# SinOncology/BreakID

Hardware: AMD Instinct MI355X
Metric: M reads/s clustered+split-scanned (higher is better)
Workload: dtype int32/u8 (+f64 sd replay)

## Files before the change

### breakid_amd/capi.py

```python
from __future__ import annotations

import ctypes as C
import math
import os
import subprocess

import numpy as np

from . import abi

_HERE = os.path.dirname(os.path.abspath(__file__))
LIB_PATH = os.path.join(_HERE, "libbreakid_hip.so")
_LIB = None


class BreakIDError(RuntimeError):
    def __init__(self, code, msg):
        super().__init__("libbreakid_hip error %d: %s" % (code, msg))
        self.code = code


def build(verbose=False):
    cmd = ["make", "-C", os.path.join(_HERE, "csrc"), "-j8"]
    r = subprocess.run(cmd, capture_output=not verbose, text=True)
    if r.returncode != 0:
        raise RuntimeError("building libbreakid_hip.so failed:\n" + (r.stdout or "")[-4000:] + (r.stderr or "")[-4000:])


EXPORTS = ["bk_init", "bk_prepare_process", "bk_free", "bk_last_error", "bk_set_stream", "bk_sync", "bk_get_stream", "bk_upload_records", "bk_records", "bk_exclude_regions", "bk_isize_stats",
           "bk_discordant_pairs", "bk_mask_and_cluster", "bk_split_evidence", "bk_cluster_summary",
           "bk_split_breakpoints", "bk_normal_support", "bk_ref_support", "bk_genotype_call", "bk_clip_support", "bk_clip_reads", "bk_base_depth", "bk_clip_rescue", "bk_junctions", "bk_junction_sides", "bk_vcf_breakend_alt", "bk_evidence", "bk_unique_support", "bk_clip_consensus", "bk_junction_fit", "bk_locus_similarity", "bk_site_complexity", "bk_window_coverage", "bk_window_context", "bk_call_windows", "bk_fusion_frame", "bk_link_calls", "bk_locus_partners", "bk_call_partner_sites", "bk_fragment_sizes", "bk_fragment_bounds", "bk_known_calls", "bk_split_junctions", "bk_split_junction_counts", "bk_debug_split_junctions", "bk_cigar_gaps", "bk_cigar_gap_counts", "bk_clip_loci", "bk_clip_locus_counts", "bk_run", "bk_fetch", "bk_timing", "bk_timing_enable", "bk_timing_touched", "bk_group_stats", "bk_qname_hash", "bk_qname_check",
           "bk_bam_open", "bk_bam_header", "bk_bam_decode", "bk_bam_close", "bk_bam_extract", "bk_bam_names_free", "bk_bam_reads", "bk_reads_free", "bk_bam_decode_device", "bk_bam_decode_device_part", "bk_bam_decode_device_ctx", "bk_bam_dev_free", "bk_feed_release_caches", "bk_debug_bgzf_inflate", "bk_debug_std_sort", "bk_debug_scan", "bk_debug_radix_sort", "bk_debug_prims_info", "bk_sort_forms", "bk_debug_sort_info", "bk_debug_ahc", "bk_debug_points", "bk_debug_points_groups", "bk_debug_cluster_info", "bk_debug_stream_info", "bk_debug_stream_blocks", "bk_debug_cigar", "bk_debug_vote", "bk_debug_region", "bk_shard_begin", "bk_shard_get_stats", "bk_shard_set_stats",
           "bk_shard_sd_local", "bk_shard_sd_finish", "bk_shard_buffer", "bk_shard_set_buffer", "bk_shard_group_sizes",
           "bk_shard_own_groups", "bk_shard_route_candidates", "bk_shard_group_keys", "bk_shard_route_pairs", "bk_shard_group_pairs", "bk_shard_bp_cov", "bk_shard_bp_vote", "bk_shard_bp_vote_slice", "bk_shard_bp_set_voted", "bk_shard_bp_depth", "bk_shard_bp_finish"]


def lib():
    global _LIB
    if _LIB is None:
        if not os.path.exists(LIB_PATH):
            raise BreakIDError(abi.BK_ERR_NO_DEVICE, "libbreakid_hip.so is not built (run __graft_entry__.build()); "
                                                     "there is no CPU fallback")
        try:
            import torch
        except Exception:
            pass
        L = C.CDLL(LIB_PATH)
        vp, u64p, dp = C.c_void_p, C.POINTER(C.c_uint64), C.POINTER(C.c_double)
        L.bk_init.argtypes = [C.c_int, vp, C.POINTER(C.c_char_p), C.c_int, C.POINTER(vp)]
        L.bk_free.argtypes = [vp]
        L.bk_last_error.restype = C.c_char_p
        L.bk_last_error.argtypes = [vp]
        L.bk_set_stream.argtypes = [vp, vp]
        L.bk_sync.argtypes = [vp]
        L.bk_upload_records.argtypes = [vp, C.POINTER(abi.Soa), C.c_int]
        L.bk_records.argtypes = [vp, C.POINTER(abi.Soa)]
        L.bk_exclude_regions.argtypes = [vp, C.POINTER(abi.Regions), u64p]
        L.bk_isize_stats.argtypes = [vp, dp, dp]
        L.bk_discordant_pairs.argtypes = [vp, C.c_int, C.c_double, u64p, C.POINTER(C.c_uint32)]
        L.bk_mask_and_cluster.argtypes = [vp, C.c_double, C.c_int, u64p]
        L.bk_split_evidence.argtypes = [vp, u64p]
        L.bk_cluster_summary.argtypes = [vp, C.c_double, u64p]
        L.bk_split_breakpoints.argtypes = [vp, C.c_double, u64p]
        L.bk_run.argtypes = [vp, C.c_int, C.c_int, dp, u64p]
        L.bk_normal_support.argtypes = [vp, vp, C.c_double, C.POINTER(vp), u64p]
        L.bk_ref_support.argtypes = [vp, vp, C.c_int, C.c_int, C.c_double, C.POINTER(vp), u64p]
        L.bk_genotype_call.argtypes = [C.c_uint32, C.c_uint32, C.POINTER(C.c_uint8), C.POINTER(C.c_uint8), C.POINTER(C.c_float)]
        L.bk_clip_support.argtypes = [vp, vp, C.c_int, C.c_int, C.c_double, C.POINTER(vp), u64p]
        L.bk_clip_reads.argtypes = [vp, vp, C.c_uint64, C.c_int, C.c_int, C.POINTER(vp), C.POINTER(vp), C.POINTER(vp)]
        L.bk_base_depth.argtypes = [vp, vp, vp, C.c_uint64, C.POINTER(vp)]
        L.bk_clip_rescue.argtypes = [vp, vp, vp, C.c_uint32] + [C.POINTER(C.c_uint32)] * 4
        L.bk_junctions.argtypes = [vp, C.POINTER(vp), u64p]
        L.bk_junction_sides.argtypes = [vp, C.POINTER(C.c_uint8), C.POINTER(C.c_uint8), C.POINTER(C.c_uint8)]
        L.bk_vcf_breakend_alt.argtypes = [C.c_char, C.c_int, C.c_char_p, C.c_uint32, C.c_int, C.c_char_p, C.c_size_t]
        L.bk_evidence.argtypes = [vp, C.POINTER(vp), u64p, C.POINTER(C.POINTER(C.c_uint64))]
        L.bk_unique_support.argtypes = [vp, C.POINTER(vp), u64p, C.POINTER(C.POINTER(C.c_uint64)), u64p]
        L.bk_clip_consensus.argtypes = [vp, C.POINTER(abi.Reads), vp, C.c_uint64, C.c_int, C.c_int, C.c_uint32, C.c_uint32, C.POINTER(vp), C.POINTER(vp), C.POINTER(vp)]
        L.bk_junction_fit.argtypes = [vp, C.POINTER(abi.RefSeq), vp, C.c_uint64, vp, C.c_uint32, C.c_uint32, C.c_uint32, C.c_uint32, C.POINTER(vp)]
        L.bk_locus_similarity.argtypes = [vp, C.POINTER(abi.RefSeq), vp, C.c_uint64, C.c_uint32, C.POINTER(vp)]
        L.bk_site_complexity.argtypes = [vp, C.POINTER(abi.RefSeq), vp, C.c_uint64, C.c_uint32, C.c_uint32, C.POINTER(vp)]
        L.bk_window_coverage.argtypes = [vp, vp, C.c_uint64, C.c_int, C.POINTER(vp)]
        L.bk_window_context.argtypes = [vp, vp, C.c_uint64, C.c_int, C.POINTER(vp)]
        L.bk_call_windows.argtypes = [vp, C.c_int, C.c_int, C.c_uint32, vp, vp]
        L.bk_fusion_frame.argtypes = [vp, C.POINTER(abi.TxModel), vp, C.c_uint64, C.POINTER(vp)]
        L.bk_link_calls.argtypes = [vp, vp, C.c_uint64, C.c_uint32, C.POINTER(vp)]
        L.bk_locus_partners.argtypes = [vp, vp, C.c_uint64, C.c_uint32, C.POINTER(vp)]
        L.bk_call_partner_sites.argtypes = [vp, C.c_double, vp]
        L.bk_fragment_sizes.argtypes = [vp, vp, C.c_uint64, C.c_int32, C.c_int32, C.POINTER(vp)]
        L.bk_fragment_bounds.argtypes = [C.c_double, C.c_double, C.POINTER(C.c_int32), C.POINTER(C.c_int32)]
        L.bk_known_calls.argtypes = [vp, vp, C.c_uint64, vp, C.c_uint64, C.c_uint32, C.POINTER(vp)]
        L.bk_split_junctions.argtypes = [vp, C.c_int, C.c_uint32, C.c_uint32, C.POINTER(vp), u64p]
        L.bk_split_junction_counts.argtypes = [vp, u64p]
        L.bk_debug_split_junctions.argtypes = [vp, C.c_int, C.c_uint32, C.c_uint32, vp, C.c_uint64, C.POINTER(vp), u64p]
        L.bk_cigar_gaps.argtypes = [vp, C.c_int, C.c_uint32, C.c_uint32, C.c_uint32, C.c_uint32, C.POINTER(vp), u64p]
        L.bk_cigar_gap_counts.argtypes = [vp, u64p]
        L.bk_clip_loci.argtypes = [vp, vp, C.c_int, C.c_int, C.c_uint32, C.c_uint32, C.c_uint32, C.POINTER(vp), u64p]
        L.bk_clip_locus_counts.argtypes = [vp, u64p]
        L.bk_fetch.argtypes = [vp, C.c_int, C.POINTER(vp), u64p, C.POINTER(C.POINTER(C.c_uint64)), C.POINTER(C.c_uint32)]
        L.bk_timing.argtypes = [vp, C.POINTER(C.POINTER(C.c_char_p)), C.POINTER(C.POINTER(C.c_float)),
                                C.POINTER(C.POINTER(C.c_uint64)), C.POINTER(C.c_int)]
        L.bk_timing_enable.argtypes = [vp, C.c_int]
        L.bk_timing_touched.argtypes = [vp, C.POINTER(C.POINTER(C.c_uint64)), C.POINTER(C.c_int)]
        L.bk_debug_std_sort.argtypes = [vp, vp, vp, C.c_uint32, vp]
        L.bk_debug_scan.argtypes = [vp, C.c_int, vp, C.c_uint64, C.c_int, vp]
        L.bk_debug_radix_sort.argtypes = [vp, vp, vp, C.c_uint64, C.c_int, C.c_int, vp, vp]
        L.bk_debug_prims_info.argtypes = [u64p]
        L.bk_sort_forms.argtypes = [vp, u64p]
        L.bk_debug_sort_info.argtypes = [vp, u64p]
        L.bk_debug_ahc.argtypes = [vp, vp, vp, C.c_uint32, C.c_double, vp, vp, C.POINTER(C.c_uint32)]
        L.bk_debug_points.argtypes = [vp, C.c_int, vp, vp, C.c_uint32, C.c_double, vp, vp, C.POINTER(C.c_uint32)]
        L.bk_debug_points_groups.argtypes = [vp, C.c_int, vp, vp, vp, C.c_uint32, C.c_double, vp, vp, vp, C.POINTER(C.c_uint32)]
        L.bk_debug_cluster_info.argtypes = [u64p]
        L.bk_debug_stream_info.argtypes = [u64p]
        L.bk_debug_stream_blocks.argtypes = [C.c_uint]
        L.bk_debug_cigar.argtypes = [vp, C.c_uint32, vp, vp, vp, vp, vp, vp, vp]
        L.bk_debug_vote.argtypes = [vp, vp, C.c_uint32, vp, C.c_uint32, C.c_int32, C.c_int32, vp]
        L.bk_debug_region.argtypes = [vp, C.c_int32, C.c_uint32, C.c_uint32, C.c_uint64, vp, C.c_uint32, C.POINTER(C.c_uint32), C.POINTER(C.c_uint32),
                                      C.POINTER(C.c_uint32)]
        L.bk_shard_begin.argtypes = [vp, C.c_uint64, C.c_int]
        L.bk_shard_get_stats.argtypes = [vp, C.POINTER(abi.ShardStats)]
        L.bk_shard_set_stats.argtypes = [vp, C.POINTER(abi.ShardStats)]
        L.bk_shard_sd_local.argtypes = [vp, u64p, C.POINTER(vp), u64p]
        L.bk_shard_sd_finish.argtypes = [vp, vp, C.c_uint64, C.c_uint64, dp, dp]
        L.bk_shard_buffer.argtypes = [vp, C.c_int, C.POINTER(vp), u64p, C.POINTER(C.c_uint32)]
        L.bk_shard_set_buffer.argtypes = [vp, C.c_int, vp, C.c_uint64]
        L.bk_shard_group_sizes.argtypes = [vp, C.POINTER(C.POINTER(C.c_uint64)), C.POINTER(C.c_uint32)]
        L.bk_shard_own_groups.argtypes = [vp, vp, C.c_uint32]
        L.bk_shard_route_candidates.argtypes = [vp, C.c_uint32, C.POINTER(vp), C.POINTER(C.POINTER(C.c_uint64))]
        L.bk_shard_group_keys.argtypes = [vp, C.POINTER(C.POINTER(C.c_uint32)), C.POINTER(C.c_uint32)]
        L.bk_shard_route_pairs.argtypes = [vp, vp, C.c_uint32, C.c_uint32, C.POINTER(vp), C.POINTER(C.POINTER(C.c_uint64))]
        L.bk_shard_group_pairs.argtypes = [vp, vp, C.c_uint64, vp, C.c_uint32]
        L.bk_shard_bp_cov.argtypes = [vp, C.c_double, C.POINTER(vp), u64p]
        L.bk_shard_bp_vote.argtypes = [vp, C.c_double, vp]
        L.bk_shard_bp_vote_slice.argtypes = [vp, C.c_double, vp, C.c_uint64, C.c_uint64, C.POINTER(vp), C.POINTER(vp)]
        L.bk_shard_bp_set_voted.argtypes = [vp, vp]
        L.bk_shard_bp_depth.argtypes = [vp, C.POINTER(vp), u64p]
        L.bk_shard_bp_finish.argtypes = [vp, vp]
        L.bk_qname_hash.restype = C.c_uint64
        L.bk_qname_hash.argtypes = [C.c_char_p, C.c_size_t]
        L.bk_qname_check.restype = C.c_uint32
        L.bk_qname_check.argtypes = [C.c_char_p, C.c_size_t]
        L.bk_bam_open.argtypes = [C.c_char_p, C.POINTER(vp), C.c_char_p, C.c_size_t]
        L.bk_bam_header.argtypes = [vp, C.POINTER(C.c_int), C.POINTER(C.POINTER(C.c_char_p)), C.POINTER(C.POINTER(C.c_uint32))]
        L.bk_bam_decode.argtypes = [vp, C.POINTER(abi.Soa), C.c_char_p, C.c_size_t]
        L.bk_bam_close.argtypes = [vp]
        L.bk_bam_extract.argtypes = [C.c_char_p, C.c_char_p, vp, C.c_uint64, C.POINTER(C.c_char_p), C.c_uint64, C.POINTER(vp), u64p, C.c_char_p, C.c_size_t]
        L.bk_bam_names_free.argtypes = [vp]
        L.bk_bam_reads.argtypes = [C.c_char_p, vp, C.c_uint64, C.POINTER(abi.Reads), C.c_char_p, C.c_size_t]
        L.bk_reads_free.argtypes = [C.POINTER(abi.Reads)]
        L.bk_reads_free.restype = None
        L.bk_bam_names_free.restype = None
        L.bk_bam_decode_device.argtypes = [C.c_char_p, C.c_int, C.POINTER(vp), C.POINTER(abi.Soa), C.POINTER(C.c_int), C.POINTER(C.POINTER(C.c_char_p)),
                                           C.POINTER(C.POINTER(C.c_uint32)), C.c_char_p, C.c_size_t]
        L.bk_bam_decode_device_part.argtypes = [C.c_char_p, C.c_int, C.c_int, C.c_int, C.POINTER(vp), C.POINTER(abi.Soa), C.POINTER(C.c_int), C.POINTER(C.POINTER(C.c_char_p)),
                                           C.POINTER(C.POINTER(C.c_uint32)), C.c_char_p, C.c_size_t]
        L.bk_bam_dev_free.argtypes = [vp]
        L.bk_feed_release_caches.argtypes = []
        L.bk_feed_release_caches.restype = None
        L.bk_bam_decode_device_ctx.argtypes = [C.c_char_p, C.c_int, C.c_int, C.POINTER(vp), C.POINTER(vp), C.POINTER(C.c_int), C.POINTER(C.POINTER(C.c_char_p)),
                                               C.POINTER(C.POINTER(C.c_uint32)), C.c_char_p, C.c_size_t]
        L.bk_debug_bgzf_inflate.argtypes = [vp, C.c_uint64, vp, C.c_uint64, C.POINTER(C.c_uint64), C.POINTER(C.c_float), C.c_char_p, C.c_size_t]
        _LIB = L
    return _LIB


MULTI_LIB_PATH = os.path.join(_HERE, "libbreakid_rccl.so")
_MULTI = None
TRANSPORT_AUTO, TRANSPORT_RCCL, TRANSPORT_LOCAL = 0, 1, 2


def multi_lib():
    global _MULTI
    if _MULTI is None:
        lib()
        if not os.path.exists(MULTI_LIB_PATH):
            raise BreakIDError(abi.BK_ERR_NO_DEVICE, "libbreakid_rccl.so is not built (run __graft_entry__.build())")
        M = C.CDLL(MULTI_LIB_PATH)
        vp, dp = C.c_void_p, C.POINTER(C.c_double)
        M.bk_multi_run.argtypes = [C.POINTER(abi.Soa), vp, C.POINTER(C.c_char_p), C.c_int, C.c_int, C.c_int, C.c_int, C.c_int, dp, C.POINTER(C.c_uint64), C.POINTER(vp),
                                   C.c_char_p, C.c_size_t]
        M.bk_multi_stats.argtypes = [vp, dp, dp, C.POINTER(vp), C.POINTER(C.c_uint32)]
        M.bk_multi_free.argtypes = [vp]
        M.bk_multi_free.restype = None
        _MULTI = M
    return _MULTI

# ... 470 lines not shown
        return np.frombuffer(buf, dtype=abi.FRAG_SIZES, count=n).copy()

    def known_calls(self, entries, sites, slop=100):
        entries = np.ascontiguousarray(entries, abi.KNOWN_ENTRY)
        sites = np.ascontiguousarray(sites, abi.KNOWN_SITE)
        assert entries.ndim == 1 and sites.ndim == 1
        n = len(sites)
        out = C.c_void_p()
        self._check(self.L.bk_known_calls(self.h, entries.ctypes.data if len(entries) else None, len(entries), sites.ctypes.data if n else None, n, slop, C.byref(out)))
        if not n:
            return np.zeros(0, abi.KNOWN_CALL)
        buf = (C.c_char * (n * abi.KNOWN_CALL.itemsize)).from_address(out.value)
        return np.frombuffer(buf, dtype=abi.KNOWN_CALL, count=n).copy()

    def split_junctions(self, mapq_min=20, tol=2, min_reads=3):
        out, n = C.c_void_p(), C.c_uint64()
        self._check(self.L.bk_split_junctions(self.h, mapq_min, tol, min_reads, C.byref(out), C.byref(n)))
        if not n.value:
            return np.zeros(0, abi.SPLIT_JUNCTION)
        buf = (C.c_char * (n.value * abi.SPLIT_JUNCTION.itemsize)).from_address(out.value)
        return np.frombuffer(buf, dtype=abi.SPLIT_JUNCTION, count=n.value).copy()

    def debug_split_junctions(self, mapq_min, tol, min_reads, clusters):
        clusters = np.ascontiguousarray(clusters, abi.CLUSTER)
        out, n = C.c_void_p(), C.c_uint64()
        self._check(self.L.bk_debug_split_junctions(self.h, mapq_min, tol, min_reads, clusters.ctypes.data if len(clusters) else None, len(clusters), C.byref(out), C.byref(n)))
        if not n.value:
            return np.zeros(0, abi.SPLIT_JUNCTION)
        buf = (C.c_char * (n.value * abi.SPLIT_JUNCTION.itemsize)).from_address(out.value)
        return np.frombuffer(buf, dtype=abi.SPLIT_JUNCTION, count=n.value).copy()

    def split_junction_counts(self):
        out = (C.c_uint64 * 6)()
        self._check(self.L.bk_split_junction_counts(self.h, out))
        return dict(zip(("tuples", "eligible", "exact", "calls", "claimed", "rounds"), (int(v) for v in out)))

    def cigar_gaps(self, mapq_min=20, min_len=20, anchor=10, tol=2, min_reads=3):
        out, n = C.c_void_p(), C.c_uint64()
        self._check(self.L.bk_cigar_gaps(self.h, mapq_min, min_len, anchor, tol, min_reads, C.byref(out), C.byref(n)))
        if not n.value:
            return np.zeros(0, abi.CIGAR_GAP)
        buf = (C.c_char * (n.value * abi.CIGAR_GAP.itemsize)).from_address(out.value)
        return np.frombuffer(buf, dtype=abi.CIGAR_GAP, count=n.value).copy()

    def cigar_gap_counts(self):
        out = (C.c_uint64 * 8)()
        self._check(self.L.bk_cigar_gap_counts(self.h, out))
        return dict(zip(("records", "eligible", "events", "beyond", "exact", "loci", "calls", "written"), (int(v) for v in out)))

    def clip_loci(self, calls=None, mapq_min=20, min_clip=10, tol=2, pair_dist=50, min_reads=3):
        out, n = C.c_void_p(), C.c_uint64()
        self._check(self.L.bk_clip_loci(self.h, calls.h if calls is not None else None, mapq_min, min_clip, tol, pair_dist, min_reads, C.byref(out), C.byref(n)))
        if not n.value:
            return np.zeros(0, abi.CLIP_LOCUS)
        buf = (C.c_char * (n.value * abi.CLIP_LOCUS.itemsize)).from_address(out.value)
        return np.frombuffer(buf, dtype=abi.CLIP_LOCUS, count=n.value).copy()

    def clip_locus_counts(self):
        out = (C.c_uint64 * 8)()
        self._check(self.L.bk_clip_locus_counts(self.h, out))
        return dict(zip(("records", "eligible", "events", "beyond", "exact", "loci", "mutual", "written"), (int(v) for v in out)))

    def run(self, qual=20, fast=True):
        w, n = C.c_double(), C.c_uint64()
        self._check(self.L.bk_run(self.h, qual, int(fast), C.byref(w), C.byref(n)))
        return w.value, n.value

    def fetch(self, stage):
        def fn(h, st, d, c, g, ng):
            return self.L.bk_fetch(h, st, d, c, g, ng)
        try:
            return abi.fetch_array(self.L, self.h, fn, stage)
        except RuntimeError:
            self._check(-1 if not self.L.bk_last_error(self.h) else abi.BK_ERR_ARG)
            raise

    def debug_std_sort(self, key, group_off):
        key = np.ascontiguousarray(key, np.uint32)
        group_off = np.ascontiguousarray(group_off, np.uint64)
        perm = np.zeros(len(key), np.uint32)
        self._check(self.L.bk_debug_std_sort(self.h, key.ctypes.data, group_off.ctypes.data, len(group_off) - 1, perm.ctypes.data))
        return perm

    def debug_scan(self, values, in_place=False):
        values = np.ascontiguousarray(values)
        assert values.ndim == 1 and values.dtype in (np.uint32, np.uint64), values.dtype
        out = np.zeros(len(values) + 1, values.dtype)
        self._check(self.L.bk_debug_scan(self.h, values.dtype.itemsize, values.ctypes.data if len(values) else None, len(values), int(in_place), out.ctypes.data))
        return out

    def debug_radix_sort(self, keys, vals, begin_bit, end_bit):
        keys = np.ascontiguousarray(keys, np.uint64)
        vals = np.ascontiguousarray(vals, np.uint32)
        assert keys.ndim == 1 and keys.shape == vals.shape
        n = len(keys)
        ko, vo = np.zeros(n, np.uint64), np.zeros(n, np.uint32)
        self._check(self.L.bk_debug_radix_sort(self.h, keys.ctypes.data if n else None, vals.ctypes.data if n else None, n, int(begin_bit), int(end_bit),
                                               ko.ctypes.data if n else None, vo.ctypes.data if n else None))
        return ko, vo

    def sort_forms(self):
        out = (C.c_uint64 * 3)()
        self._check(self.L.bk_sort_forms(self.h, out))
        return tuple(int(v) for v in out)

    SORT_INFO = ("FIN_MAX", "HEAP_BIG_MIN", "HEAP_RANKED_MAX", "HEAP_LARGE", "SVC_WIDE_MIN", "F2_HB", "F2_EXT", "HEAP_PAD", "SJ_MAX_WIDE", "SJ_MAX_NARROW",
                 "cap32", "max_heap", "n_heap")

    def debug_sort_info(self):
        out = (C.c_uint64 * len(self.SORT_INFO))()
        self._check(self.L.bk_debug_sort_info(self.h, out))
        return dict(zip(self.SORT_INFO, (int(v) for v in out)))

    def debug_ahc(self, x, y, w):
        x = np.ascontiguousarray(x, np.uint32)
        y = np.ascontiguousarray(y, np.uint32)
        n = len(x)
        idx = np.zeros(max(n, 1), np.uint32)
        cl = np.zeros(max(n, 1), np.int32)
        m = C.c_uint32()
        self._check(self.L.bk_debug_ahc(self.h, x.ctypes.data, y.ctypes.data, n, float(w), idx.ctypes.data, cl.ctypes.data, C.byref(m)))
        return idx[:m.value].copy(), cl[:m.value].copy()

    def debug_points(self, mode, x, y, w):
        x = np.ascontiguousarray(x, np.uint32)
        y = np.ascontiguousarray(y, np.uint32)
        n = len(x)
        idx = np.zeros(max(n, 1), np.uint32)
        cl = np.zeros(max(n, 1), np.int32)
        m = C.c_uint32()
        self._check(self.L.bk_debug_points(self.h, {"mask": 0, "iso": 1, "fast": 2}[mode], x.ctypes.data, y.ctypes.data, n, float(w), idx.ctypes.data,
                                           cl.ctypes.data, C.byref(m)))
        return idx[:m.value].copy(), cl[:m.value].copy()

    def debug_points_groups(self, mode, x, y, group_off, w):
        x = np.ascontiguousarray(x, np.uint32)
        y = np.ascontiguousarray(y, np.uint32)
        group_off = np.ascontiguousarray(group_off, np.uint64)
        n = len(x)
        assert len(y) == n and len(group_off) >= 1 and int(group_off[-1]) == n
        idx = np.zeros(2 * n + 1, np.uint32)
        cl = np.zeros(2 * n + 1, np.int32)
        goff = np.zeros(len(group_off), np.uint64)
        m = C.c_uint32()
        self._check(self.L.bk_debug_points_groups(self.h, {"mask": 0, "iso": 1, "fast": 2}[mode], x.ctypes.data, y.ctypes.data, group_off.ctypes.data,
                                                  len(group_off) - 1, float(w), idx.ctypes.data, cl.ctypes.data, goff.ctypes.data, C.byref(m)))
        return idx[:m.value].copy(), cl[:m.value].copy(), goff

    def debug_cigar(self, rows):
        kind = np.asarray([1 if r[0] == "b" else 0 for r in rows], np.uint8)
        c1 = bytearray()
        o1 = [0]
        for r in rows:
            while r[0] == "b" and len(c1) % 4:
                c1 += b"\0"
                o1[-1] = len(c1)
            c1 += np.asarray(r[1], np.uint32).tobytes() if r[0] == "b" else r[1].encode()
            o1.append(len(c1))
        c2 = bytearray()
        o2 = [0]
        for r in rows:
            c2 += r[2].encode()
            o2.append(len(c2))
        o1a, o2a = np.asarray(o1, np.uint32), np.asarray(o2, np.uint32)
        b1 = np.frombuffer(bytes(c1) + b"\0" * 16, np.uint8)
        b2 = np.frombuffer(bytes(c2) + b"\0" * 16, np.uint8)
# ... 271 lines not shown
```

### breakid_amd/csrc/api.hip

```cpp
#include <algorithm>
#include <cmath>
#include <limits>
#include <cstring>
#include <numeric>

#include "bk_common.h"
#include "prims.h"
#include "stream.h"
#include "join.h"
#include "cluster.h"
#include "bp.h"
#include "normal.h"
#include "genotype.h"
#include "clip.h"
#include "junction.h"
#include "evidence.h"
#include "unique.h"
#include "consensus.h"
#include "jfit.h"
#include "locsim.h"
#include "seqcx.h"
#include "coverage.h"
#include "context.h"
#include "frame.h"
// ... 2348 lines not shown
int bk_shard_bp_cov(bk_ctx *ctx, double w, void **cov_dev, uint64_t *n)
{
  return guarded(ctx, [&] {
    uint32_t *cov = bp_cov_partial(rec_view(ctx), ctx->clusters_ptr(), ctx->n_clusters, w, (int) ctx->hc.max_span, ctx->bb, ctx->st);
    HIP_CHECK(hipStreamSynchronize(ctx->st));
    if (cov_dev) *cov_dev = cov;
    if (n) *n = 2 * ctx->n_clusters;
  });
}

int bk_shard_bp_vote(bk_ctx *ctx, double w, const void *cov_total_dev)
{
  return guarded(ctx, [&] {
    ensure_splits_sorted(ctx);
    bp_vote(ctx->d_split.get<bk_split>(), ctx->hc.n_split, ctx->clusters_ptr(), ctx->n_clusters, w, (int) ctx->hc.max_span, (const uint32_t *) cov_total_dev,
            ctx->d_hdr.get<int32_t>(), ctx->bb, ctx->st);
    HIP_CHECK(hipStreamSynchronize(ctx->st));
  });
}

int bk_shard_bp_vote_slice(bk_ctx *ctx, double w, const void *cov_total_dev, uint64_t lo, uint64_t hi, void **clusters_dev, void **voted_dev)
{
  return guarded(ctx, [&] {
    if (lo > hi || hi > ctx->n_clusters || !clusters_dev || !voted_dev) throw bk_error(BK_ERR_ARG, "bk_shard_bp_vote_slice: bad range");
    ensure_splits_sorted(ctx);
    bp_vote(ctx->d_split.get<bk_split>(), ctx->hc.n_split, ctx->clusters_ptr() + lo, hi - lo, w, (int) ctx->hc.max_span,
            cov_total_dev ? (const uint32_t *) cov_total_dev + 2 * lo : nullptr, ctx->d_hdr.get<int32_t>(), ctx->bb, ctx->st);
    HIP_CHECK(hipStreamSynchronize(ctx->st));
    *clusters_dev = ctx->clusters_ptr() + lo;
    *voted_dev = ctx->bb.voted.p;
  });
}

int bk_shard_bp_set_voted(bk_ctx *ctx, const void *voted_all_dev)
{
  return guarded(ctx, [&] {
    uint32_t *v = ctx->bb.voted.as<uint32_t>(ctx->n_clusters + 1);
    if (ctx->n_clusters && voted_all_dev != v)
      HIP_CHECK(hipMemcpyAsync(v, voted_all_dev, ctx->n_clusters * 4, hipMemcpyDeviceToDevice, ctx->st));
    HIP_CHECK(hipStreamSynchronize(ctx->st));
  });
}

int bk_shard_bp_depth(bk_ctx *ctx, void **depth_dev, uint64_t *n)
{
  return guarded(ctx, [&] {
    uint32_t *d = bp_depth_partial(rec_view(ctx), ctx->clusters_ptr(), ctx->n_clusters, (int) ctx->hc.max_span, ctx->bb, ctx->st);
    HIP_CHECK(hipStreamSynchronize(ctx->st));
    if (depth_dev) *depth_dev = d;
    if (n) *n = 2 * ctx->n_clusters;
  });
}

int bk_shard_bp_finish(bk_ctx *ctx, const void *depth_total_dev)
{
  return guarded(ctx, [&] {
    bp_finish(ctx->clusters_ptr(), ctx->n_clusters, (const uint32_t *) depth_total_dev, ctx->bb, ctx->st);
    HIP_CHECK(hipStreamSynchronize(ctx->st));
  });
}

int bk_debug_std_sort(bk_ctx *ctx, const uint32_t *key, const uint64_t *group_off, uint32_t n_groups, uint32_t *perm_out)
{
  return guarded(ctx, [&] {
    if (!key || !group_off || !perm_out) throw bk_error(BK_ERR_ARG, "bk_debug_std_sort: null argument");
    const uint64_t n = group_off[n_groups];
    DevBuf dk, dp, dgof, dgoff;
    std::vector<uint32_t> gof(n), iota(n);
    for (uint32_t g = 0; g < n_groups; ++g)
      for (uint64_t p = group_off[g]; p < group_off[g + 1]; ++p) gof[p] = g;
    std::iota(iota.begin(), iota.end(), 0u);
    HIP_CHECK(hipMemcpy(dk.as<uint32_t>(n + 1), key, n * 4, hipMemcpyHostToDevice));
    HIP_CHECK(hipMemcpy(dp.as<uint32_t>(n + 1), iota.data(), n * 4, hipMemcpyHostToDevice));
    HIP_CHECK(hipMemcpy(dgof.as<uint32_t>(n + 1), gof.data(), n * 4, hipMemcpyHostToDevice));
    HIP_CHECK(hipMemcpy(dgoff.as<uint64_t>((uint64_t) n_groups + 1), group_off, ((uint64_t) n_groups + 1) * 8, hipMemcpyHostToDevice));
    uint64_t max_group = 0;
    for (uint32_t g = 0; g < n_groups; ++g) max_group = std::max<uint64_t>(max_group, group_off[g + 1] - group_off[g]);
    ctx->stage.debug_sort(ctx->device, ctx->st, dk.get<uint32_t>(), dp.get<uint32_t>(), dgof.get<uint32_t>(), dgoff.get<uint64_t>(), n_groups, n, max_group);
    HIP_CHECK(hipMemcpyAsync(perm_out, dp.get<uint32_t>(), n * 4, hipMemcpyDeviceToHost, ctx->st));
    HIP_CHECK(hipStreamSynchronize(ctx->st));
  });
}

int bk_debug_scan(bk_ctx *ctx, int elem_bytes, const void *in, uint64_t n, int in_place, void *out)
{
  return guarded(ctx, [&] {
    if (elem_bytes != 4 && elem_bytes != 8) throw bk_error(BK_ERR_ARG, "bk_debug_scan: elem_bytes must be 4 or 8");
    if (!out || (n && !in)) throw bk_error(BK_ERR_ARG, "bk_debug_scan: null argument");
    auto run = [&](auto zero) {
      using T = decltype(zero);
      T *d_in = ctx->dbg_in.as<T>(n + 1);
      T *d_out = in_place ? d_in : ctx->dbg_out.as<T>(n + 1);
      HIP_CHECK(hipMemsetAsync(d_out, 0xA5, (n + 1) * sizeof(T), ctx->st));
      if (n) HIP_CHECK(hipMemcpyAsync(d_in, in, n * sizeof(T), hipMemcpyHostToDevice, ctx->st));
      prims::exclusive_scan<T>(d_in, d_out, n, ctx->dbg_radix.scan_tmp, ctx->st);
      HIP_CHECK(hipMemcpyAsync(out, d_out, (n + 1) * sizeof(T), hipMemcpyDeviceToHost, ctx->st));
      HIP_CHECK(hipStreamSynchronize(ctx->st));
    };
    if (elem_bytes == 4)
      run(uint32_t(0));
    else
      run(uint64_t(0));
  });
}

int bk_debug_radix_sort(bk_ctx *ctx, const uint64_t *keys, const uint32_t *vals, uint64_t n, int begin_bit, int end_bit, uint64_t *keys_out, uint32_t *vals_out)
{
  return guarded(ctx, [&] {
    if (n && (!keys || !vals || !keys_out || !vals_out)) throw bk_error(BK_ERR_ARG, "bk_debug_radix_sort: null argument");
    if (begin_bit < 0 || end_bit > 64) throw bk_error(BK_ERR_ARG, "bk_debug_radix_sort: bits outside [0, 64]");
    prims::radix_check_count(n);
    if (!n) return;
    prims::RadixBufs &rb = ctx->dbg_radix;
    uint64_t *dk = ctx->dbg_in.as<uint64_t>(n);
    uint32_t *dv = ctx->dbg_vals.as<uint32_t>(n);
    HIP_CHECK(hipMemsetAsync(rb.keys_alt.as<uint64_t>(n), 0xA5, n * 8, ctx->st));
    HIP_CHECK(hipMemsetAsync(rb.vals_alt.as<uint32_t>(n), 0xA5, n * 4, ctx->st));
    HIP_CHECK(hipMemcpyAsync(dk, keys, n * 8, hipMemcpyHostToDevice, ctx->st));
    HIP_CHECK(hipMemcpyAsync(dv, vals, n * 4, hipMemcpyHostToDevice, ctx->st));
    uint64_t *ko = nullptr;
    uint32_t *vo = nullptr;
    prims::radix_sort_pairs(dk, dv, n, begin_bit, end_bit, rb, ctx->st, &ko, &vo);
    HIP_CHECK(hipMemcpyAsync(keys_out, ko, n * 8, hipMemcpyDeviceToHost, ctx->st));
    HIP_CHECK(hipMemcpyAsync(vals_out, vo, n * 4, hipMemcpyDeviceToHost, ctx->st));
    HIP_CHECK(hipStreamSynchronize(ctx->st));
  });
}

int bk_debug_prims_info(uint64_t out[4])
{
  if (!out) return BK_ERR_ARG;
  out[0] = prims::BLOCK;
  out[1] = prims::SCAN_TILE;
  out[2] = prims::SCAN_ONE_MAX;
  out[3] = prims::RS_TILE;
  return BK_OK;
}

int bk_sort_forms(bk_ctx *ctx, uint64_t out[3])
{
  return guarded(ctx, [&] {
    if (!out) throw bk_error(BK_ERR_ARG, "bk_sort_forms: null output");
    ctx->stage.sort_forms(out);
  });
}

int bk_debug_sort_info(bk_ctx *ctx, uint64_t out[13])
{
  return guarded(ctx, [&] {
    if (!out) throw bk_error(BK_ERR_ARG, "bk_debug_sort_info: null output");
    static_assert(SORT_INFO_WORDS == 11, "bk_debug_sort_info: eleven words of the build, two of the last sort");
    std_sort_info(out);
    const SortEmuBufs &se = ctx->stage.cb().se;
    out[11] = se.last_heap[0];
    out[12] = se.last_heap[1];
  });
}

int bk_debug_ahc(bk_ctx *ctx, const uint32_t *x, const uint32_t *y, uint32_t n, double w, uint32_t *idx_out, int32_t *cluster_out, uint32_t *n_out)
{
  return guarded(ctx, [&] {
    if (!x || !y || !idx_out || !cluster_out || !n_out) throw bk_error(BK_ERR_ARG, "bk_debug_ahc: null argument");
    std::vector<bk_pair> hp(n);
    for (uint32_t i = 0; i < n; ++i)
    {
      memset(&hp[i], 0, sizeof(bk_pair));
// ... 440 lines not shown
```

### breakid_amd/csrc/cluster.h

```cpp
#pragma once
#include "bk_common.h"
#include "prims.h"
#include "sortemu.h"

constexpr uint32_t FW_TILE = 1024, FW_LEVELS = 10;
static_assert((1ull << FW_LEVELS) >= FW_TILE, "k_fw_exit / k_fw_mark: FW_LEVELS rounds of doubling must cover a tile of one-element windows");
static_assert(FW_LEVELS < 32 && FW_TILE <= 1024 && FW_TILE < 0xFFFFu, "FW_TILE is a workgroup size and its positions are uint16");

struct PairList
{
  uint64_t n = 0;
  uint32_t ng = 0;
  DevBuf idx;
  DevBuf gof;
  DevBuf goff;
  uint64_t total(hipStream_t st) const;
};

struct ClusterBufs
{
  std::vector<uint32_t> heavy_x, heavy_y;
  bool observe = false;
  uint64_t max_group_bound = 0;
  DevBuf key, perm, tmp, cnt, off, off2, idx2, gof2, goff2, jump, mark, apos, kid, kprev2, k1, k2, pk, knum, clfull, small, scan_tmp;
  SortEmuBufs se;
  prims::RadixBufs radix;
};

void remove_isolated_all(const bk_pair *pairs, const uint32_t *gof0, const uint64_t *gstart, uint32_t ng, uint64_t n, double w, PairList &L, ClusterBufs &b, hipStream_t st,
                         const uint32_t *drop_group = nullptr);
void remove_isolated_begin(const bk_pair *pairs, const uint32_t *gof0, const uint64_t *gstart, uint32_t ng, uint64_t n, double w, PairList &L, ClusterBufs &b, hipStream_t st,
                           const uint32_t *drop_group = nullptr, const uint64_t *gstart_host = nullptr, const uint8_t *keep_host = nullptr);
void remove_isolated_end(const bk_pair *pairs, PairList &L, ClusterBufs &b, hipStream_t st);
void list_subset_ranges(const PairList &src, const uint64_t *src_goff_host, const uint8_t *keep_host, PairList &dst, hipStream_t st);
void drop_small_groups(PairList &L, ClusterBufs &b, hipStream_t st);
void fast_cluster_all(const bk_pair *pairs, PairList &L, double w, DevBuf &cluster_out, ClusterBufs &b, hipStream_t st);
void merge_lists_many(const PairList *const *lists, const uint32_t *const *cls, int K, PairList &out, DevBuf *cl_out, hipStream_t st);
void debug_mask_list(const bk_pair *pairs, PairList &L, long dist, ClusterBufs &b, hipStream_t st);
```

### breakid_amd/csrc/cluster.hip

```cpp
#include "bk_common.h"
#include "prims.h"
#include "sortemu.h"
#include "cluster.h"

namespace
{
constexpr uint32_t END = 0xFFFFFFFFu;

__global__ __launch_bounds__(256) void k_iota(uint32_t *__restrict__ a, uint64_t n)
{
  uint64_t i = (uint64_t) blockIdx.x * blockDim.x + threadIdx.x;
  if (i < n) a[i] = (uint32_t) i;
}
__global__ __launch_bounds__(256) void k_gather_key(const bk_pair *__restrict__ pairs, const uint32_t *__restrict__ idx, uint64_t n, int use_y, uint32_t *__restrict__ key)
{
  uint64_t p = (uint64_t) blockIdx.x * blockDim.x + threadIdx.x;
  if (p < n) key[p] = use_y ? pairs[idx[p]].y : pairs[idx[p]].x;
}
__global__ __launch_bounds__(256) void k_gather_u32(const uint32_t *__restrict__ src, const uint32_t *__restrict__ perm, uint64_t n, uint32_t *__restrict__ dst)
{
  uint64_t p = (uint64_t) blockIdx.x * blockDim.x + threadIdx.x;
  if (p < n) dst[p] = src[perm[p]];
}

// ... 206 lines not shown
{
  uint64_t p = (uint64_t) blockIdx.x * blockDim.x + threadIdx.x;
  if (p >= n || !first[p]) return;
  uint64_t gs = goff[gof[p]];
  knum[uid[p]] = fscan[p] - fscan[gs] + 1;
}
__global__ __launch_bounds__(256) void k_cluster_of(const uint32_t *__restrict__ uid, const uint32_t *__restrict__ knum, const uint32_t *__restrict__ keep, uint64_t n,
                                                    uint32_t *__restrict__ cl)
{
  uint64_t p = (uint64_t) blockIdx.x * blockDim.x + threadIdx.x;
  if (p < n) cl[p] = keep[p] ? knum[uid[p]] : 0u;
}
__global__ void k_group_small(const uint64_t *__restrict__ goff, uint32_t ng, uint32_t *__restrict__ small)
{
  uint32_t g = blockIdx.x * blockDim.x + threadIdx.x;
  if (g < ng) small[g] = (goff[g + 1] - goff[g]) < 2 ? 1u : 0u;
}
__global__ __launch_bounds__(256) void k_drop_small(const uint32_t *__restrict__ gof, const uint32_t *__restrict__ small, uint64_t n, uint32_t *__restrict__ keep)
{
  uint64_t p = (uint64_t) blockIdx.x * blockDim.x + threadIdx.x;
  if (p < n) keep[p] = small[gof[p]] ? 0u : 1u;
}
}

uint64_t PairList::total(hipStream_t st) const
{
  uint64_t t = 0;
  if (ng == 0) return 0;
  HIP_CHECK(hipMemcpyAsync(&t, goff.get<uint64_t>() + ng, 8, hipMemcpyDeviceToHost, st));
  HIP_CHECK(hipStreamSynchronize(st));
  return t;
}

static inline unsigned nb(uint64_t n) { return cdiv(n ? n : 1, 256); }
static void filter_groups(PairList &L, const uint32_t *drop, ClusterBufs &b, hipStream_t st);

static void sort_list(const bk_pair *pairs, PairList &L, int use_y, uint32_t **extra, int n_extra, ClusterBufs &b, hipStream_t st)
{
  if (L.n == 0) return;
  uint32_t *key = b.key.as<uint32_t>(L.n), *perm = b.perm.as<uint32_t>(L.n);
  hipLaunchKernelGGL(k_gather_key, dim3(nb(L.n)), dim3(256), 0, st, pairs, L.idx.get<uint32_t>(), L.n, use_y, key);
  hipLaunchKernelGGL(k_iota, dim3(nb(L.n)), dim3(256), 0, st, perm, L.n);
  b.se.heavy = b.observe ? (use_y ? &b.heavy_y : &b.heavy_x) : nullptr;
  std_sort_groups(key, perm, L.gof.get<uint32_t>(), L.goff.get<uint64_t>(), L.ng, L.n, b.se, st);
  b.se.heavy = nullptr;
  uint32_t *tmp = b.tmp.as<uint32_t>(L.n);
  auto apply = [&](uint32_t *arr) {
    hipLaunchKernelGGL(k_gather_u32, dim3(nb(L.n)), dim3(256), 0, st, arr, perm, L.n, tmp);
    HIP_CHECK(hipMemcpyAsync(arr, tmp, L.n * 4, hipMemcpyDeviceToDevice, st));
  };
  apply(L.idx.get<uint32_t>());
  for (int k = 0; k < n_extra; ++k) apply(extra[k]);
}

static void mask_list(const bk_pair *pairs, PairList &L, long dist, ClusterBufs &b, hipStream_t st)
{
  if (L.n == 0) return;
  uint32_t *cnt = b.cnt.as<uint32_t>(L.n + 1);
  hipLaunchKernelGGL(k_mask_count, dim3(nb(L.n)), dim3(256), 0, st, pairs, L.idx.get<uint32_t>(), L.gof.get<uint32_t>(), L.goff.get<uint64_t>(), L.n, dist, cnt);
  uint32_t *off = b.off.as<uint32_t>(L.n + 1);
  prims::exclusive_scan<uint32_t>(cnt, off, L.n, b.scan_tmp, st);
  uint32_t total = 0;
  HIP_CHECK(hipMemcpyAsync(&total, off + L.n, 4, hipMemcpyDeviceToHost, st));
  HIP_CHECK(hipStreamSynchronize(st));
  uint32_t *oidx = b.idx2.as<uint32_t>((uint64_t) total + 1), *ogof = b.gof2.as<uint32_t>((uint64_t) total + 1);
  uint64_t *ogoff = b.goff2.as<uint64_t>((uint64_t) L.ng + 1);
  hipLaunchKernelGGL(k_expand, dim3(nb(L.n)), dim3(256), 0, st, cnt, off, L.idx.get<uint32_t>(), L.gof.get<uint32_t>(), L.n, oidx, ogof);
  hipLaunchKernelGGL(k_new_goff, dim3(cdiv(L.ng + 1, 256)), dim3(256), 0, st, off, L.goff.get<uint64_t>(), L.ng, L.n, ogoff);
  std::swap(L.idx, b.idx2);
  std::swap(L.gof, b.gof2);
  std::swap(L.goff, b.goff2);
  L.n = total;
}

void remove_isolated_all(const bk_pair *pairs, const uint32_t *gof0, const uint64_t *gstart, uint32_t ng, uint64_t n, double w, PairList &L, ClusterBufs &b, hipStream_t st,
                         const uint32_t *drop_group)
{
  remove_isolated_begin(pairs, gof0, gstart, ng, n, w, L, b, st, drop_group, nullptr, nullptr);
  remove_isolated_end(pairs, L, b, st);
}

void remove_isolated_end(const bk_pair *pairs, PairList &L, ClusterBufs &b, hipStream_t st)
{
  if (L.n == 0 || L.ng == 0) return;
  sort_list(pairs, L, 0, nullptr, 0, b, st);
}

namespace
{
__global__ __launch_bounds__(256) void k_subset_list(const uint64_t *__restrict__ gstart, const uint64_t *__restrict__ goff, uint32_t ng, uint64_t n_list,
                                                     uint32_t *__restrict__ idx, uint32_t *__restrict__ gof)
{
  const uint64_t p = (uint64_t) blockIdx.x * blockDim.x + threadIdx.x;
  if (p >= n_list) return;
  uint32_t lo = 0, hi = ng;
  while (hi - lo > 1)
  {
    const uint32_t m = (lo + hi) >> 1;
    if (goff[m] <= p) lo = m; else hi = m;
  }
  idx[p] = (uint32_t) (gstart[lo] + (p - goff[lo]));
  gof[p] = lo;
}
}
namespace
{
__global__ __launch_bounds__(256) void k_subset_of_list(const uint32_t *__restrict__ src_idx, const uint64_t *__restrict__ src_goff, const uint64_t *__restrict__ goff, uint32_t ng,
                                                        uint64_t n_list, uint32_t *__restrict__ idx, uint32_t *__restrict__ gof)
{
  const uint64_t p = (uint64_t) blockIdx.x * blockDim.x + threadIdx.x;
  if (p >= n_list) return;
  uint32_t lo = 0, hi = ng;
  while (hi - lo > 1)
  {
    const uint32_t m = (lo + hi) >> 1;
    if (goff[m] <= p) lo = m; else hi = m;
  }
  idx[p] = src_idx[src_goff[lo] + (p - goff[lo])];
  gof[p] = lo;
}
}
void list_subset_ranges(const PairList &src, const uint64_t *src_goff_host, const uint8_t *keep_host, PairList &dst, hipStream_t st)
{
  const uint32_t ng = src.ng;
  std::vector<uint64_t> goff((size_t) ng + 1, 0);
  for (uint32_t g = 0; g < ng; ++g) goff[g + 1] = goff[g] + (keep_host[g] ? src_goff_host[g + 1] - src_goff_host[g] : 0);
  dst.n = goff[ng];
  dst.ng = ng;
  uint32_t *idx = dst.idx.as<uint32_t>(dst.n + 1), *gof = dst.gof.as<uint32_t>(dst.n + 1);
  uint64_t *dgoff = dst.goff.as<uint64_t>((uint64_t) ng + 1);
  HIP_CHECK(hipMemcpyAsync(dgoff, goff.data(), ((size_t) ng + 1) * 8, hipMemcpyHostToDevice, st));
  HIP_CHECK(hipStreamSynchronize(st));
  if (dst.n) hipLaunchKernelGGL(k_subset_of_list, dim3(nb(dst.n)), dim3(256), 0, st, src.idx.get<uint32_t>(), src.goff.get<uint64_t>(), dgoff, ng, dst.n, idx, gof);
}

void list_of_groups(const uint64_t *gstart_dev, const uint64_t *gstart_host, const uint8_t *keep_host, uint32_t ng, PairList &L, hipStream_t st)
{
  std::vector<uint64_t> goff((size_t) ng + 1, 0);
  for (uint32_t g = 0; g < ng; ++g) goff[g + 1] = goff[g] + (keep_host[g] ? gstart_host[g + 1] - gstart_host[g] : 0);
  L.n = goff[ng];
  L.ng = ng;
  uint32_t *idx = L.idx.as<uint32_t>(L.n + 1), *gof = L.gof.as<uint32_t>(L.n + 1);
  uint64_t *dgoff = L.goff.as<uint64_t>((uint64_t) ng + 1);
  HIP_CHECK(hipMemcpyAsync(dgoff, goff.data(), ((size_t) ng + 1) * 8, hipMemcpyHostToDevice, st));
  HIP_CHECK(hipStreamSynchronize(st));
  if (L.n) hipLaunchKernelGGL(k_subset_list, dim3(nb(L.n)), dim3(256), 0, st, gstart_dev, dgoff, ng, L.n, idx, gof);
}

void remove_isolated_begin(const bk_pair *pairs, const uint32_t *gof0, const uint64_t *gstart, uint32_t ng, uint64_t n, double w, PairList &L, ClusterBufs &b, hipStream_t st,
                           const uint32_t *drop_group, const uint64_t *gstart_host, const uint8_t *keep_host)
{
  if (gstart_host && keep_host)
  {
    if (n == 0 || ng == 0)
    {
      L.n = 0;
      L.ng = ng;
      (void) L.idx.as<uint32_t>(1);
      (void) L.gof.as<uint32_t>(1);
      (void) L.goff.as<uint64_t>((uint64_t) ng + 1);
      return;
    }
    list_of_groups(gstart, gstart_host, keep_host, ng, L, st);
  }
  else
  {
    L.n = n;
    L.ng = ng;
// ... 186 lines not shown
```

### breakid_amd/csrc/lanes.h

```cpp
#pragma once
#include <functional>
#include <memory>

#include "join.h"
#include "cluster.h"
#include "ahc.h"

void stage_set_hw_queues(int n);

struct StageInput
{
  int device;
  hipStream_t st;
  const JoinResult &jr;
  const std::vector<uint64_t> &gstart_host;
  const std::vector<uint8_t> &own_groups;
  std::function<void(const char *name, const std::function<void()> &body)> timed;
};

struct ClusterStage
{
  SortService svc;
  std::vector<hipEvent_t> svc_probe;
  int svc_late = 0;
  bool svc_refused = false;
  struct Lane
  {
    ClusterBufs cb;
    PairList list, iso;
    DevBuf d_cluster;
    hipStream_t st = nullptr;
    ~Lane()
    {
      if (st) (void) hipStreamDestroy(st);
    }
  };
  std::vector<std::unique_ptr<Lane>> lanes;
  ClusterBufs &cb() { return lanes[0]->cb; }
  AhcBufs ab;
  PairList list;
  DevBuf d_cluster, iso_idx, iso_goff;
  uint64_t iso_n = 0;
  PairList lane_mid, lane_iso_m;
  DevBuf d_drop;

  ClusterStage() { lanes.emplace_back(new Lane()); }
  void run(const StageInput &in, double w, int fast);
  void sort_forms(uint64_t out[3]) const;
  void debug_sort(int device, hipStream_t st, uint32_t *key, uint32_t *idx, const uint32_t *gof, const uint64_t *goff, uint32_t ng, uint64_t n, uint64_t max_group);
};
```

### breakid_amd/csrc/lanes.hip

```cpp
#include <algorithm>
#include <atomic>
#include <chrono>
#include <cmath>
#include <cstdio>
#include <numeric>
#include <thread>
#include <dirent.h>

#include "lanes.h"

static int g_hw_queues_at_init = 0;
void stage_set_hw_queues(int n) { g_hw_queues_at_init = n; }

static bool sort_service_on()
{
  static const bool on = !(getenv("BREAKID_SORT_SERVICE") && atoi(getenv("BREAKID_SORT_SERVICE")) == 0);
  return on;
}
constexpr int LANE_STREAMS_MAX = 4;
constexpr int SVC_STAGE_QUEUES = LANE_STREAMS_MAX + 3;
static bool lane_service(int fast) { return sort_service_on() && fast && g_hw_queues_at_init >= SVC_STAGE_QUEUES; }
static int stage_queues() { return std::max(1, g_hw_queues_at_init - 1); }
static int lanes_wanted(bool svc)
{
  const char *env = getenv("BREAKID_GROUP_LANES");
  static const int want_svc = env ? atoi(env) : 12;
  if (svc) return want_svc < 1 ? 1 : (want_svc > 26 ? 26 : want_svc);
  static const int want = env ? atoi(env) : std::min(4, stage_queues());
  return want < 1 ? 1 : (want > 26 ? 26 : want);
}
static bool lanes_apply(const StageInput &in, int fast)
{
  static const uint64_t min_pairs = getenv("BREAKID_LANES_MIN_PAIRS") ? strtoull(getenv("BREAKID_LANES_MIN_PAIRS"), nullptr, 10) : (1ull << 20);
  uint32_t large = 0;
  const uint64_t big = std::max<uint64_t>(2, min_pairs >> 6);
  for (uint32_t g = 0; g < in.jr.n_groups && g + 1 < in.gstart_host.size(); ++g) large += in.gstart_host[g + 1] - in.gstart_host[g] >= big ? 1u : 0u;
  const bool yes = lanes_wanted(lane_service(fast)) >= 2 && fast && in.jr.n_groups >= 4 && in.jr.n_pairs >= min_pairs && large >= 2;
  if (yes)
  {
    static bool told = false;
    const int K = lanes_wanted(lane_service(fast));
    if (!told && !lane_service(fast) && K > stage_queues() && bk_debug("lanes"))
    {
      told = true;
      fprintf(stderr, "[breakid] GPU_MAX_HW_QUEUES=%d: the lanes of chromosome-pair groups (bk_mask_and_cluster) and their heap kernels will share hardware queues "
                        "(BREAKID_GROUP_LANES=1: one pass)\n", g_hw_queues_at_init);
    }
  }
  return yes;
}

__global__ void k_svc_probe() {}
static int kfd_compute_queues(int device)
{
  char bus[64] = {0};
  if (hipDeviceGetPCIBusId(bus, (int) sizeof bus, device) != hipSuccess) return -1;
  unsigned dom = 0, b = 0, d = 0, f = 0;
  if (sscanf(bus, "%x:%x:%x.%x", &dom, &b, &d, &f) != 4) return -1;
  const unsigned long want_loc = (b << 8) | (d << 3) | f;
  auto read_file = [](const std::string &path, std::string &out) {
    FILE *fp = fopen(path.c_str(), "r");
    if (!fp) return false;
    char buf[4096];
    const size_t n = fread(buf, 1, sizeof buf - 1, fp);
    fclose(fp);
    buf[n] = 0;
    out = buf;
    return true;
  };
  auto list_dir = [](const std::string &path, std::vector<std::string> &names) {
    DIR *dp = opendir(path.c_str());
    if (!dp) return false;
    while (dirent *e = readdir(dp))
      if (e->d_name[0] != '.') names.push_back(e->d_name);
    closedir(dp);
    return true;
  };
  unsigned long gpu_id = 0;
  {
    std::vector<std::string> nodes;
    if (!list_dir("/sys/class/kfd/kfd/topology/nodes", nodes)) return -1;
    for (const std::string &n : nodes)
    {
      std::string props, id;
      const std::string base = "/sys/class/kfd/kfd/topology/nodes/" + n;
      if (!read_file(base + "/properties", props) || !read_file(base + "/gpu_id", id)) continue;
      unsigned long loc = ~0ul, domain = ~0ul;
      size_t p = props.find("location_id ");
      if (p != std::string::npos) loc = strtoul(props.c_str() + p + 12, nullptr, 10);
      p = props.find("domain ");
      if (p != std::string::npos) domain = strtoul(props.c_str() + p + 7, nullptr, 10);
      if (loc == want_loc && (domain == ~0ul || domain == dom) && strtoul(id.c_str(), nullptr, 10) != 0) gpu_id = strtoul(id.c_str(), nullptr, 10);
    }
  }
  if (!gpu_id) return -1;
  std::vector<std::string> procs;
  if (!list_dir("/sys/class/kfd/kfd/proc", procs)) return -1;
  int total = 0;
  for (const std::string &pid : procs)
  {
    std::vector<std::string> qs;
    const std::string qdir = "/sys/class/kfd/kfd/proc/" + pid + "/queues";
    if (!list_dir(qdir, qs)) continue;
    for (const std::string &q : qs)
    {
      std::string g, t;
      if (!read_file(qdir + "/" + q + "/gpuid", g) || !read_file(qdir + "/" + q + "/type", t)) continue;
      if (strtoul(g.c_str(), nullptr, 10) == gpu_id && strtoul(t.c_str(), nullptr, 10) == 0) ++total;
    }
  }
  return total;
}
// ... 90 lines not shown
    return ok && took < 0.003;
  }
  void set(SortService *s)
  {
    for (auto &l : cs.lanes)
    {
      l->cb.se.svc = s;
      l->cb.se.svc_slot = 0xFFFFFFFFu;
    }
  }
  void finish()
  {
    if (!on) return;
    on = false;
    set(nullptr);
    hipError_t e = hipStreamSynchronize(st);
    for (auto &l : cs.lanes)
      if (l->st && e == hipSuccess) e = hipStreamSynchronize(l->st);
    cs.svc.stop();
    device_turn.unlock();
    if (e != hipSuccess) throw bk_error(BK_ERR_HIP, std::string("sort service: ") + hipGetErrorString(e));
  }
  ~SvcStage()
  {
    try
    {
      finish();
    }
    catch (const bk_error &)
    {
    }
  }
};

static void snapshot_list(const PairList &L, DevBuf &idx, DevBuf *gof, DevBuf &goff, hipStream_t st)
{
  uint32_t *ii = idx.as<uint32_t>(L.n + 1), *ig = gof ? gof->as<uint32_t>(L.n + 1) : nullptr;
  uint64_t *io = goff.as<uint64_t>((uint64_t) L.ng + 1);
  if (L.n) HIP_CHECK(hipMemcpyAsync(ii, L.idx.get<uint32_t>(), L.n * 4, hipMemcpyDeviceToDevice, st));
  if (L.n && ig) HIP_CHECK(hipMemcpyAsync(ig, L.gof.get<uint32_t>(), L.n * 4, hipMemcpyDeviceToDevice, st));
  if (L.ng) HIP_CHECK(hipMemcpyAsync(io, L.goff.get<uint64_t>(), ((uint64_t) L.ng + 1) * 8, hipMemcpyDeviceToDevice, st));
}
static void cluster_list(const bk_pair *pairs, PairList &L, double w, int fast, DevBuf &cl, ClusterBufs &cb, AhcBufs &ab, hipStream_t st)
{
  if (fast)
    fast_cluster_all(pairs, L, w, cl, cb, st);
  else
    ahc_cluster_all(pairs, L, w, cl, ab, cb, st);
}

using LanePlan = std::vector<int>;
static LanePlan plan_owned(const StageInput &in)
{
  const uint32_t ng = in.jr.n_groups;
  const bool owned_only = !in.own_groups.empty();
  if (owned_only && in.own_groups.size() != ng) throw bk_error(BK_ERR_ARG, "bk_shard_own_groups: group count changed");
  LanePlan p(ng, 0);
  for (uint32_t g = 0; owned_only && g < ng; ++g)
    if (!in.own_groups[g]) p[g] = -1;
  return p;
}
static LanePlan plan_blind(const StageInput &in, int K)
{
  const uint32_t ng = in.jr.n_groups;
  std::vector<uint32_t> order(ng);
  std::iota(order.begin(), order.end(), 0u);
  auto size_of = [&](uint32_t g) { return in.gstart_host[g + 1] - in.gstart_host[g]; };
  std::stable_sort(order.begin(), order.end(), [&](uint32_t a, uint32_t b) { return size_of(a) > size_of(b); });
  constexpr double wexp = 2.0;
  LanePlan p = plan_owned(in);
  std::vector<double> load(K, 0.0);
  for (uint32_t i = 0; i < ng; ++i)
  {
    const uint32_t g = order[i];
    if (p[g] < 0) continue;
    int l = 0;
    for (int k = 1; k < K; ++k)
      if (load[k] < load[l]) l = k;
    load[l] += std::pow((double) size_of(g), wexp);
    p[g] = l;
  }
  return p;
}
static LanePlan plan_observed(const std::vector<uint64_t> &sizes, const std::vector<uint32_t> &hx, const std::vector<uint32_t> &hy, int K)
{
  const uint32_t ng = (uint32_t) sizes.size();
  constexpr double per_pair = 0.001;
  auto heap_cost = [](uint32_t m) { return (double) m + (m > 40947u ? 1.0 * (double) (m - 40947u) : 0.0); };
  std::vector<uint32_t> order(ng);
  std::iota(order.begin(), order.end(), 0u);
  auto chain = [&](uint32_t g) { return heap_cost(hx[g]) + heap_cost(hy[g]); };
  std::stable_sort(order.begin(), order.end(), [&](uint32_t a, uint32_t b) {
    const double ca = chain(a), cb = chain(b);
    return ca != cb ? ca > cb : sizes[a] > sizes[b];
  });
  LanePlan p(ng, 0);
  std::vector<double> mx(K, 0.0), my(K, 0.0), pairs(K, 0.0);
  auto cost = [&](int l) { return mx[l] + my[l] + per_pair * pairs[l]; };
  for (uint32_t g : order)
  {
    int best = 0;
    double best_cost = 0;
    for (int l = 0; l < K; ++l)
    {
      const double c = std::max(mx[l], heap_cost(hx[g])) + std::max(my[l], heap_cost(hy[g])) + per_pair * (pairs[l] + (double) sizes[g]);
      if (l == 0 || c < best_cost || (c == best_cost && cost(l) < cost(best)))
      {
        best = l;
        best_cost = c;
      }
    }
    mx[best] = std::max(mx[best], heap_cost(hx[g]));
    my[best] = std::max(my[best], heap_cost(hy[g]));
    pairs[best] += (double) sizes[g];
    p[g] = best;
  }
  if (bk_debug("lanes"))
    for (int l = 0; l < K; ++l)
    {
      fprintf(stderr, "[lanes] lane %d: max heap x %.0f y %.0f, %.0f pairs, cost %.0f; heavy groups:", l, mx[l], my[l], pairs[l], cost(l));
      for (uint32_t g = 0; g < ng; ++g)
        if (p[g] == l && (hx[g] || hy[g])) fprintf(stderr, " %u(%u,%u)", g, hx[g], hy[g]);
      fprintf(stderr, "\n");
    }
  return p;
}
static uint32_t *upload_drop(const LanePlan &p, int K, DevBuf &buf, hipStream_t st)
{
  const size_t row = p.size() + 1;
  std::vector<uint32_t> drop((size_t) K * row, 0u);
  for (int l = 0; l < K; ++l)
    for (size_t g = 0; g + 1 < row; ++g) drop[(size_t) l * row + g] = p[g] == l ? 0u : 1u;
  uint32_t *d = buf.as<uint32_t>(drop.size() + 1);
  HIP_CHECK(hipMemcpyAsync(d, drop.data(), drop.size() * 4, hipMemcpyHostToDevice, st));
  HIP_CHECK(hipStreamSynchronize(st));
  return d;
}

static void group_lanes(ClusterStage &cs, const StageInput &in, double w, int fast)
{
  const uint32_t ng = in.jr.n_groups;
  static const bool dbg = bk_debug("lanes");
  auto make_lanes = [&](int K, int S) {
    while ((int) cs.lanes.size() < K)
    {
      cs.lanes.emplace_back(new ClusterStage::Lane());
      cs.lanes.back()->cb.max_group_bound = cs.cb().max_group_bound;
    }
    for (int k = 1; k < S; ++k)
      if (!cs.lanes[k]->st) HIP_CHECK(hipStreamCreateWithFlags(&cs.lanes[k]->st, hipStreamNonBlocking));
  };
  bool use_svc = sort_service_on() && fast;
  if (use_svc && !lane_service(fast))
  {
    use_svc = false;
    tell_no_service();
    if (bk_debug("lanes")) fprintf(stderr, "[lanes] %d hardware queues, the sort service needs %d: not started\n", g_hw_queues_at_init, SVC_STAGE_QUEUES);
  }
  int K = lanes_wanted(use_svc);
  int S = use_svc ? std::max(1, std::min(LANE_STREAMS_MAX, K)) : K;
  make_lanes(K, S);
  std::vector<hipStream_t> stage_streams{in.st};
  for (int k = 1; k < S; ++k) stage_streams.push_back(cs.lanes[k]->st);
  SvcStage svc_stage(cs, in.device, in.st, use_svc, in.jr.n_pairs + 2ull * ng + 4096, cs.cb().max_group_bound, stage_streams);
  if (use_svc && !svc_stage.on)
  {
    use_svc = false;
    K = lanes_wanted(false);
    S = K;
    make_lanes(K, S);
  }
  if (!use_svc && bk_debug("lanes"))
  {
    fprintf(stderr, "[lanes] launch path: %d lanes, 1 stream each, %d hardware queues\n", K, g_hw_queues_at_init);
    fprintf(stderr, "[lanes] sorts as task dispatches on the lane streams\n");
  }
  auto lane = [&](int l) -> ClusterStage::Lane & { return *cs.lanes[l]; };
  auto lane_st = [&](int l) { const int k = l % S; return k == 0 ? in.st : cs.lanes[k]->st; };
  uint32_t *drop_base = nullptr;
  auto lane_drop = [&](int l) { return drop_base + (size_t) l * ((size_t) ng + 1); };
  std::vector<std::vector<uint8_t>> keep(K, std::vector<uint8_t>(ng, 0));
  auto upload_plan = [&](const LanePlan &p) {
    for (int l = 0; l < K; ++l)
      for (uint32_t g = 0; g < ng; ++g) keep[l][g] = p[g] == l ? 1 : 0;
    drop_base = upload_drop(p, K, cs.d_drop, in.st);
  };
  auto in_lanes = [&](auto body) {
    std::vector<std::string> err(K);
    std::vector<int> code(K, BK_OK);
    const auto t_start = std::chrono::steady_clock::now();
    auto guarded_body = [&](int l) {
      try
      {
        body(l);
        HIP_CHECK(hipStreamSynchronize(lane_st(l)));
        if (dbg)
          fprintf(stderr, "[lanes] lane %d done after %.2f ms\n", l, std::chrono::duration<double, std::milli>(std::chrono::steady_clock::now() - t_start).count());
      }
      catch (const bk_error &e)
      {
        code[l] = e.code;
        err[l] = e.msg;
      }
    };
    std::vector<std::thread> th;
    for (int l = 1; l < K; ++l)
      th.emplace_back([&, l] {
        (void) hipSetDevice(in.device);
        guarded_body(l);
      });
    guarded_body(0);
    for (std::thread &t : th) t.join();
    for (int l = 0; l < K; ++l)
      if (code[l] != BK_OK) throw bk_error(code[l], err[l]);
  };
  auto merge_all = [&](PairList ClusterStage::Lane::*which, PairList &out, DevBuf *cl_out) {
    std::vector<const PairList *> ls(K);
    std::vector<const uint32_t *> cls(K);
    for (int l = 0; l < K; ++l)
    {
      ls[l] = &(lane(l).*which);
      cls[l] = lane(l).d_cluster.get<uint32_t>();
    }
    merge_lists_many(ls.data(), cl_out ? cls.data() : nullptr, K, out, cl_out, in.st);
  };
  const bk_pair *pairs = in.jr.pairs;
  auto mask_lane = [&](int l, bool observe) {
    ClusterBufs &cb = lane(l).cb;
    if (observe)
    {
      cb.heavy_x.assign(ng, 0u);
      cb.heavy_y.assign(ng, 0u);
      cb.observe = true;
      cb.se.heavy_all = false;
    }
    remove_isolated_begin(pairs, in.jr.gof, in.jr.gstart, ng, in.jr.n_pairs, w, lane(l).list, cb, lane_st(l), lane_drop(l), in.gstart_host.data(), keep[l].data());
    if (observe) cb.heavy_x.assign(ng, 0u);
    remove_isolated_end(pairs, lane(l).list, cb, lane_st(l));
    if (observe) cb.observe = false;
  };
  auto cluster_lane = [&](int l) {
    PairList &L = lane(l).list, &iso = lane(l).iso;
    iso.n = L.n;
    iso.ng = L.ng;
    snapshot_list(L, iso.idx, &iso.gof, iso.goff, lane_st(l));
    cluster_list(pairs, L, w, fast, lane(l).d_cluster, lane(l).cb, cs.ab, lane_st(l));
  };
  const auto tp0 = std::chrono::steady_clock::now();
  auto phase = [&](const char *what) {
    if (dbg) fprintf(stderr, "[lanes] %s at %.2f ms\n", what, std::chrono::duration<double, std::milli>(std::chrono::steady_clock::now() - tp0).count());
  };
  upload_plan(plan_blind(in, K));
  phase("plan uploaded");
  if (use_svc)
    in_lanes([&](int l) {
      mask_lane(l, false);
      cluster_lane(l);
    });
  else
  {
    in_lanes([&](int l) { mask_lane(l, true); });
    PairList &mid = cs.lane_mid;
    merge_all(&ClusterStage::Lane::list, mid, nullptr);
    std::vector<uint64_t> goff_h((size_t) ng + 1);
    HIP_CHECK(hipMemcpyAsync(goff_h.data(), mid.goff.get<uint64_t>(), ((size_t) ng + 1) * 8, hipMemcpyDeviceToHost, in.st));
    HIP_CHECK(hipStreamSynchronize(in.st));
    std::vector<uint64_t> sizes(ng);
    std::vector<uint32_t> hx(ng, 0u), hy(ng, 0u);
    for (uint32_t g = 0; g < ng; ++g) sizes[g] = goff_h[g + 1] - goff_h[g];
    for (int l = 0; l < K; ++l)
      for (uint32_t g = 0; g < ng; ++g)
      {
        hx[g] = std::max(hx[g], lane(l).cb.heavy_x[g]);
        hy[g] = std::max(hy[g], lane(l).cb.heavy_y[g]);
      }
    upload_plan(plan_observed(sizes, hx, hy, K));
    in_lanes([&](int l) {
      list_subset_ranges(mid, goff_h.data(), keep[l].data(), lane(l).list, lane_st(l));
      cluster_lane(l);
    });
  }
  phase("lanes done");
  svc_stage.finish();
  phase("service stopped");
  if (use_svc && bk_debug("lanes")) fprintf(stderr, "[svc] tasks: %u wide, %u narrow\n", cs.svc.stats[0], cs.svc.stats[1]);
  PairList &iso_m = cs.lane_iso_m;
  merge_all(&ClusterStage::Lane::iso, iso_m, nullptr);
  merge_all(&ClusterStage::Lane::list, cs.list, &cs.d_cluster);
  HIP_CHECK(hipStreamSynchronize(in.st));
  phase("lists merged");
  cs.iso_n = iso_m.n;
  std::swap(cs.iso_idx, iso_m.idx);
  std::swap(cs.iso_goff, iso_m.goff);
}

void ClusterStage::run(const StageInput &in, double w, int fast)
{
  uint64_t mg = 0;
  for (uint32_t g = 0; g < in.jr.n_groups && g + 1 < in.gstart_host.size(); ++g) mg = std::max<uint64_t>(mg, in.gstart_host[g + 1] - in.gstart_host[g]);
  for (auto &l : lanes) l->cb.max_group_bound = mg;
  if (lanes_apply(in, fast))
  {
    in.timed("mask_and_cluster_lanes", [&] { group_lanes(*this, in, w, fast); });
    return;
  }
  SvcStage svc_stage(*this, in.device, in.st, true, in.jr.n_pairs + 2ull * in.jr.n_groups + 4096, cb().max_group_bound, {in.st});
  in.timed("remove_isolated", [&] {
    const uint32_t *drop = in.own_groups.empty() ? nullptr : upload_drop(plan_owned(in), 1, d_drop, in.st);
    remove_isolated_all(in.jr.pairs, in.jr.gof, in.jr.gstart, in.jr.n_groups, in.jr.n_pairs, w, list, cb(), in.st, drop);
  });
  iso_n = list.n;
  snapshot_list(list, iso_idx, nullptr, iso_goff, in.st);
  if (!fast) svc_stage.finish();
  in.timed(fast ? "fast_cluster" : "ahc_cluster", [&] { cluster_list(in.jr.pairs, list, w, fast, d_cluster, cb(), ab, in.st); });
  svc_stage.finish();
}

void ClusterStage::sort_forms(uint64_t out[3]) const
{
  out[0] = out[1] = out[2] = 0;
  for (const auto &l : lanes)
    for (int k = 0; k < 2; ++k) out[k] += l->cb.se.sorts[k];
}

void ClusterStage::debug_sort(int device, hipStream_t st, uint32_t *key, uint32_t *idx, const uint32_t *gof, const uint64_t *goff, uint32_t ng, uint64_t n, uint64_t max_group)
{
  SvcStage svc_stage(*this, device, st, true, n + 2ull * ng + 4096, max_group, {st});
  std_sort_groups(key, idx, gof, goff, ng, n, cb().se, st);
  svc_stage.finish();
}
```

### breakid_amd/csrc/sortemu.h

```cpp
#pragma once
#include "bk_common.h"
#include <vector>
#include <atomic>

struct SortService
{
  DevBuf ctl, slots[2], seq[2], jobs, dbg, pos[2];
  uint32_t pos_cap[2] = {0, 0};
  uint32_t cap[2] = {0, 0};
  hipStream_t st[2] = {nullptr, nullptr}, quit_stream = nullptr, st_copy = nullptr;
  uint32_t *quit_host = nullptr;
  uint32_t *quit_dev = nullptr;
  uint32_t cap32 = 0;
  uint32_t quit_word = 0, starts = 0;
  size_t wide_lds = 0;
  bool running = false;
  std::atomic<uint32_t> next_slot{0};
  uint32_t stats[8] = {};
  void start(uint64_t n_bound, uint64_t max_group, hipStream_t after);
  bool narrow_running(double seconds) const;
  void stop();
  uint32_t new_slot() { return next_slot.fetch_add(1u); }
  ~SortService();
  SortService() = default;
  SortService(const SortService &) = delete;
  SortService &operator=(const SortService &) = delete;
};

struct SortEmuBufs
{
  SortService *svc = nullptr;
  uint32_t svc_slot = 0xFFFFFFFFu, svc_epoch = 0;
  DevBuf heap_scratch, scratch32, scratch32b, rk_a, rk_b, chk_key0, chk_cnt, chk_bad;
  std::vector<uint32_t> *heavy = nullptr;
  bool heavy_all = false;
  DevBuf tj_ctl, tj_jobs, tj_slots[2], tj_seq[2], tj_pos[2], tj_heavy, tj_trace;
  uint32_t tj_cap[2] = {0, 0}, tj_epoch = 0;
  bool tj_ready = false;
  uint64_t sorts[2] = {0, 0};
  uint32_t last_heap[2] = {0, 0};
  SortEmuBufs() = default;
  SortEmuBufs(const SortEmuBufs &) = delete;
  SortEmuBufs &operator=(const SortEmuBufs &) = delete;
};

void std_sort_groups(uint32_t *key, uint32_t *idx, const uint32_t *gof, const uint64_t *goff, uint32_t ng, uint64_t n, SortEmuBufs &b, hipStream_t st);

constexpr int SORT_INFO_WORDS = 11;
void std_sort_info(uint64_t out[SORT_INFO_WORDS]);
```

### breakid_amd/csrc/sortemu.hip

```cpp
#include "bk_common.h"
#include "sortemu.h"
#include <vector>
#include <mutex>
#include <algorithm>
#include <cstdio>
#include <chrono>
#include <thread>
#include <cstdlib>

namespace
{
typedef __attribute__((address_space(1))) uint32_t gu32_t;
__device__ __forceinline__ void st_through(uint32_t *p, uint32_t v) { __hip_atomic_store((gu32_t *) p, v, __ATOMIC_RELAXED, __HIP_MEMORY_SCOPE_AGENT); }
constexpr uint32_t FIN_MAX = 2048;
constexpr uint32_t HEAP_BIG_MIN = 4096;

typedef unsigned long long hent;
__device__ __forceinline__ uint32_t hkey(hent e) { return (uint32_t) (e >> 32); }

struct E64
{
  typedef hent T;
  static __device__ __forceinline__ uint32_t key(T e) { return (uint32_t) (e >> 32); }
};
// ... 1022 lines not shown
        fprintf(stderr, "[svc]   %s workgroups by last state (1 polling, 5 took a task, 9 left):", kind ? "narrow" : "wide");
        for (auto &kv : hist) fprintf(stderr, " %u:%d", kv.first, kv.second);
        fprintf(stderr, "; first ones (state, polls, time of the last poll in 10 ns, how it left 6 error 7 quit 8 timeout):");
        for (uint32_t w = 0; w < 6 && w < n; ++w) fprintf(stderr, " [%u %u %u %u]", d[4 * (w + 4096 * kind)], d[4 * (w + 4096 * kind) + 1], d[4 * (w + 4096 * kind) + 2], d[4 * (w + 4096 * kind) + 3]);
        fprintf(stderr, "\n");
      }
    }
    uint32_t sq[4] = {};
    HIP_CHECK(hipMemcpy(sq, seq[1].get<uint32_t>(), sizeof sq, hipMemcpyDeviceToHost));
    fprintf(stderr, "[svc] tasks %u wide / %u narrow; workgroups started %u / %u, left on their own %u / %u, odd quit words read %u; error %u; wide queue head %u tail %u, narrow queue head %u tail %u (seq %u %u %u %u); job 0: remaining %u done %u heaps %u (longest %u)\n",
            stats[0], stats[1], stats[2], stats[3], stats[4], stats[5], stats[6], h[0], c[0], c[32], c[64], c[96], sq[0], sq[1], sq[2], sq[3], j0.remaining, j0.done, j0.n_heap, j0.max_heap);
  }
  if (h[0]) throw bk_error(h[0] & 2u ? BK_ERR_LIMIT : BK_ERR_HIP, "sort service: task error " + std::to_string(h[0]) + " (2 = ring overflow, 4 = a job timed out, 8 = a cut outside its segment, 16 = a task in the wrong queue, 32 = a node beyond the position lists, 64 = the finisher); first failing task: code " + std::to_string(h[8]) + ", " + std::to_string(h[9]) + " " + std::to_string(h[10]) + " " + std::to_string(h[11]));
}
SortService::~SortService()
{
  if (running)
  {
    running = false;
    if (quit_host && st_copy)
    {
      __atomic_store_n(quit_host, quit_word, __ATOMIC_SEQ_CST);
      (void) hipMemcpyAsync(ctl.get<uint32_t>() + 192, quit_host, 4, hipMemcpyHostToDevice, st_copy);
    }
    if (quit_stream) hipLaunchKernelGGL(k_svc_quit, dim3(1), dim3(1), 0, quit_stream, ctl.get<uint32_t>() + 192, quit_word);
    for (int k = 0; k < 2; ++k)
      if (st[k]) (void) hipStreamSynchronize(st[k]);
    DeferredFrees::end();
  }
  for (int k = 0; k < 2; ++k)
    if (st[k]) (void) hipStreamDestroy(st[k]);
  if (st_copy) (void) hipStreamDestroy(st_copy);
  if (quit_host) (void) hipHostFree(quit_host);
}

static void window_sorts(uint32_t *key, uint32_t *idx, const uint32_t *gof, uint32_t n, hipStream_t st);

static void std_sort_groups_svc(uint32_t *key, uint32_t *idx, const uint32_t *gof, const uint64_t *goff, uint32_t ng, uint32_t n, SortEmuBufs &b, hipStream_t st)
{
  SortService &S = *b.svc;
  if (b.svc_slot == 0xFFFFFFFFu)
  {
    b.svc_slot = S.new_slot();
    if (b.svc_slot >= SVC_MAX_JOBS) throw bk_error(BK_ERR_LIMIT, "sort service: more than 64 callers");
  }
  SvcJob d = {};
  d.key = key;
  d.idx = idx;
  d.hscratch = b.heap_scratch.as<hent>((uint64_t) n + HEAP_PAD);
  d.scratch32 = b.scratch32.as<uint32_t>((uint64_t) n + HEAP_PAD);
  d.scratch32b = b.scratch32b.as<uint32_t>((uint64_t) n + HEAP_PAD);
  d.rka = b.rk_a.as<unsigned long long>((uint64_t) n + HEAP_PAD);
  d.rkb = b.rk_b.as<unsigned long long>((uint64_t) n + HEAP_PAD);
  d.epoch = (b.svc_epoch++ % 0xFFFFFu) + 1u;
  const SvcParams P = svc_params(S);
  hipLaunchKernelGGL(k_svc_submit, dim3(1), dim3(256), 0, st, P, d, b.svc_slot, goff, ng);
  HIP_CHECK(hipGetLastError());
  {
    volatile const uint32_t *done = S.quit_host + SVC_H_DONE + b.svc_slot, *err = S.quit_host + SVC_H_ERROR;
    const auto t0 = std::chrono::steady_clock::now();
    for (uint32_t spins = 0; *done != d.epoch; ++spins)
    {
      if (*err != 0u)
        throw bk_error(BK_ERR_HIP, "sort service: a task failed (error " + std::to_string(*err) + "; first failing task: code " + std::to_string(err[1]) + ", " + std::to_string(err[2]) + " " + std::to_string(err[3]) + " " + std::to_string(err[4]) + ")");
      if ((spins & 1023u) == 1023u)
      {
        if (std::chrono::duration<double>(std::chrono::steady_clock::now() - t0).count() > 20.0) throw bk_error(BK_ERR_HIP, "sort service: a job did not finish");
        std::this_thread::yield();
      }
      else
        __builtin_ia32_pause();
    }
  }
  if (bk_debug("svc"))
  {
    SvcJob j;
    HIP_CHECK(hipMemcpy(&j, S.jobs.get<SvcJob>() + b.svc_slot, sizeof j, hipMemcpyDeviceToHost));
    fprintf(stderr, "[svc] slot %u sort %u: %u elements in %u groups; partitions and finisher done after %.3f ms, job after %.3f ms; %u elements in heaps, the longest %u, the heap that ended last %u elements in %.3f ms\n", b.svc_slot,
            b.svc_epoch, n, ng, (double) (j.t_parts - j.t_submit) * 1e-5, (double) (j.t_done - j.t_submit) * 1e-5, j.n_heap, j.max_heap, (uint32_t) j.last_heap, (double) (j.last_heap >> 32) * 1e-5);
  }
  window_sorts(key, idx, gof, n, st);
}

static void std_sort_groups_tasks(uint32_t *key, uint32_t *idx, const uint32_t *gof, const uint64_t *goff, uint32_t ng, uint32_t n, SortEmuBufs &b, hipStream_t st, const uint32_t *key0)
{
  static size_t dyn_lds = 0;
  static uint32_t cap32 = 0;
  static std::once_flag once;
  std::call_once(once, [] {
    const WideLds w = wide_lds_split(reinterpret_cast<const void *>(k_sort_job));
    dyn_lds = w.dyn_lds;
    cap32 = w.cap32;
    if (dyn_lds < SJ_TEAMS * SJ_TEAM_LDS) throw bk_error(BK_ERR_HIP, "k_sort_job: the narrow teams do not fit the LDS");
    HIP_CHECK(hipFuncSetAttribute(reinterpret_cast<const void *>(k_sort_job), hipFuncAttributeMaxDynamicSharedMemorySize, (int) dyn_lds));
  });
  std::vector<uint64_t> go((size_t) ng + 1);
  HIP_CHECK(hipMemcpyAsync(go.data(), goff, go.size() * 8, hipMemcpyDeviceToHost, st));
  HIP_CHECK(hipStreamSynchronize(st));
  uint64_t max_group = 0;
  for (uint32_t g = 0; g < ng; ++g) max_group = std::max<uint64_t>(max_group, go[g + 1] - go[g]);
  const uint32_t n_wide = std::min<uint32_t>(SJ_MAX_WIDE, std::max<uint32_t>(1, cdiv(n, 1u << 16)));
  const uint32_t n_narrow = std::min<uint32_t>(SJ_MAX_NARROW, std::max<uint32_t>(1, cdiv(n, 1u << 16)));
  SjParams S = {};
  SvcParams &P = S.P;
  {
    auto pow2 = [](uint64_t v) {
      uint32_t c = 1024;
      while (c < v && c < (1u << 30)) c <<= 1;
      return c;
    };
    const uint32_t want[2] = {pow2((uint64_t) n / HEAP_BIG_MIN + 4096), pow2((uint64_t) n / 16 + 4096)};
    for (int k = 0; k < 2; ++k)
      if (want[k] > b.tj_cap[k])
      {
        b.tj_cap[k] = want[k];
        b.tj_ready = false;
      }
    uint32_t *ctl = b.tj_ctl.as<uint32_t>(SJ_C_WORDS);
    for (int k = 0; k < 2; ++k)
    {
      P.q[k].head = ctl + 64 * k;
      P.q[k].tail = ctl + 64 * k + 32;
      P.q[k].slots = b.tj_slots[k].as<SvcTask>(b.tj_cap[k]);
      P.q[k].seq = b.tj_seq[k].as<uint32_t>(b.tj_cap[k]);
      P.q[k].mask = b.tj_cap[k] - 1;
      P.q[k].release = 1u;
    }
    P.error = ctl + SJ_C_ERROR;
    P.stats = ctl + SJ_C_STATS;
    P.quit_d = ctl + SJ_C_QUIT;
    P.host = ctl + SJ_C_HOST;
    P.jobs = b.tj_jobs.as<SvcJob>(SVC_MAX_JOBS);
    P.cap32 = cap32;
    P.quit_word = 0u;
    P.timeout_ticks = SJ_TIMEOUT_TICKS;
    P.pos_cap[0] = (uint32_t) std::max<uint64_t>(max_group, SVC_WIDE_MIN) + 64;
    P.pos_cap[1] = SVC_WIDE_MIN + 64;
    P.pos[0] = b.tj_pos[0].as<uint32_t>(2ull * P.pos_cap[0] * n_wide);
    P.pos[1] = b.tj_pos[1].as<uint32_t>(2ull * P.pos_cap[1] * n_narrow * SJ_TEAMS);
    P.dbg = nullptr;
    S.n_wide = n_wide;
    S.live = ctl + SJ_C_LIVE;
    S.gof = gof;
    S.heavy_min = b.heavy_all ? FIN_MAX : HEAP_RANKED_MIN;
    if (b.heavy)
    {
      S.heavy = b.tj_heavy.as<uint32_t>(ng);
      HIP_CHECK(hipMemsetAsync(S.heavy, 0, (size_t) ng * 4, st));
    }
  }
  static const bool dbg = bk_debug("svc");
  if (dbg) S.trace = b.tj_trace.as<unsigned long long>(8);
  if (!b.tj_ready)
  {
    HIP_CHECK(hipMemsetAsync(b.tj_ctl.p, 0, SJ_C_WORDS * 4, st));
    hipLaunchKernelGGL(k_svc_reset, dim3(cdiv(std::max(b.tj_cap[0], b.tj_cap[1]), 256)), dim3(256), 0, st, P);
    b.tj_ready = true;
  }
  SvcJob d = {};
  d.key = key;
  d.idx = idx;
  d.hscratch = b.heap_scratch.as<hent>((uint64_t) n + HEAP_PAD);
  d.scratch32 = b.scratch32.as<uint32_t>((uint64_t) n + HEAP_PAD);
  d.scratch32b = b.scratch32b.as<uint32_t>((uint64_t) n + HEAP_PAD);
  d.rka = b.rk_a.as<unsigned long long>((uint64_t) n + HEAP_PAD);
  d.rkb = b.rk_b.as<unsigned long long>((uint64_t) n + HEAP_PAD);
  d.epoch = (b.tj_epoch++ % 0xFFFFFu) + 1u;
  const SvcJobLds J = {d.key, d.idx, nullptr, nullptr, d.hscratch, d.scratch32, d.scratch32b, d.rka, d.rkb, P.jobs, d.epoch << 8};
  hipLaunchKernelGGL(k_sort_job_submit, dim3(1), dim3(256), 0, st, S, d, goff, ng);
  hipLaunchKernelGGL(k_sort_job, dim3(n_wide + n_narrow), dim3(1024), dyn_lds, st, S, J);
  HIP_CHECK(hipGetLastError());
  ++b.sorts[1];
  if (key0) sort_check("after the task dispatch", key, idx, key0, n, goff, ng, st, b);
  window_sorts(key, idx, gof, n, st);
  uint32_t h[16] = {};
  HIP_CHECK(hipMemcpyAsync(h, P.error, 12 * 4, hipMemcpyDeviceToHost, st));
  std::vector<uint32_t> hv;
  if (S.heavy)
  {
    hv.resize(ng);
    HIP_CHECK(hipMemcpyAsync(hv.data(), S.heavy, (size_t) ng * 4, hipMemcpyDeviceToHost, st));
  }
  unsigned long long tr[8] = {};
  if (S.trace) HIP_CHECK(hipMemcpyAsync(tr, S.trace, 5 * 8, hipMemcpyDeviceToHost, st));
  SvcJob j = {};
  HIP_CHECK(hipMemcpyAsync(&j, P.jobs, sizeof j, hipMemcpyDeviceToHost, st));
  HIP_CHECK(hipStreamSynchronize(st));
  b.last_heap[0] = j.max_heap;
  b.last_heap[1] = j.n_heap;
  if (h[0] || j.remaining != 0u)
  {
    b.tj_ready = false;
    throw bk_error(h[0] & 2u ? BK_ERR_LIMIT : BK_ERR_HIP, "sort task dispatch: task error " + std::to_string(h[0]) + " (2 = ring overflow, 4 = no progress for 1 s, 8 = a cut outside its segment, 16 = a task in the wrong queue, 32 = a node beyond the position lists, 64 = the finisher), " + std::to_string(j.remaining) + " elements not final; first failing task: code " + std::to_string(h[8]) + ", " + std::to_string(h[9]) + " " + std::to_string(h[10]) + " " + std::to_string(h[11]));
  }
  if (S.heavy)
  {
    if (b.heavy->size() < ng) b.heavy->resize(ng, 0u);
    for (uint32_t g = 0; g < ng; ++g) (*b.heavy)[g] = std::max((*b.heavy)[g], hv[g]);
  }
  if (S.trace)
  {
    const double t0 = (double) tr[0];
    const uint32_t hm = (uint32_t) (tr[1] >> 40);
    const unsigned long long hs = tr[1] & 0xFFFFFFFFFFull, base = tr[0] & ~0xFFFFFFFFFFull;
    unsigned long long hstart = base | hs;
    if (hstart < tr[0]) hstart += 1ull << 40;
    fprintf(stderr, "[svc] task dispatch %u: %u elements in %u groups on %u wide + %u narrow workgroups; longest heap %u elements started %.3f ms after the dispatch and took %.3f ms; partitions and finisher done after %.3f ms, job after %.3f ms; %u elements in heaps, the longest %u\n",
            d.epoch, n, ng, n_wide, n_narrow, hm, hm ? ((double) hstart - t0) * 1e-5 : 0.0, hm ? (double) (tr[2] & 0xFFFFFFFFFFull) * 1e-5 : 0.0, tr[3] ? ((double) tr[3] - t0) * 1e-5 : 0.0, ((double) tr[4] - t0) * 1e-5, j.n_heap, j.max_heap);
  }
}

void std_sort_groups(uint32_t *key, uint32_t *idx, const uint32_t *gof, const uint64_t *goff, uint32_t ng, uint64_t n64, SortEmuBufs &b, hipStream_t st)
{
  if (n64 == 0 || ng == 0) return;
  if (n64 > 0x7FFFFFF0ull) throw bk_error(BK_ERR_LIMIT, "std_sort_groups: more than 2^31 pairs");
  const uint32_t n = (uint32_t) n64;
  if (b.svc && b.svc->running)
  {
    ++b.sorts[0];
    b.last_heap[0] = b.last_heap[1] = 0xFFFFFFFFu;
    std_sort_groups_svc(key, idx, gof, goff, ng, n, b, st);
    return;
  }
  static const bool chk = bk_debug("sortcheck");
  DevBuf &chk_key0 = b.chk_key0;
  uint32_t *key0 = nullptr;
  if (chk)
  {
    key0 = chk_key0.as<uint32_t>(n);
    std::vector<uint32_t> hk(n), hx(n), k0(n);
    HIP_CHECK(hipStreamSynchronize(st));
    HIP_CHECK(hipMemcpy(hk.data(), key, (size_t) n * 4, hipMemcpyDeviceToHost));
    HIP_CHECK(hipMemcpy(hx.data(), idx, (size_t) n * 4, hipMemcpyDeviceToHost));
    for (uint32_t i = 0; i < n; ++i)
      if (hx[i] < n) k0[hx[i]] = hk[i];
    HIP_CHECK(hipMemcpy(key0, k0.data(), (size_t) n * 4, hipMemcpyHostToDevice));
    sort_check("at entry", key, idx, key0, n, goff, ng, st, b);
  }
  if (const char *dump = getenv("BK_DEBUG_SORT_DUMP"))
  {
    static int call = 0;
    if (call < 5)
    {
      std::vector<uint64_t> go((size_t) ng + 1);
      std::vector<uint32_t> kk(n);
      HIP_CHECK(hipStreamSynchronize(st));
      HIP_CHECK(hipMemcpy(go.data(), goff, ((size_t) ng + 1) * 8, hipMemcpyDeviceToHost));
      HIP_CHECK(hipMemcpy(kk.data(), key, (size_t) n * 4, hipMemcpyDeviceToHost));
      char name[512];
      snprintf(name, sizeof name, "%s.%d.keys.u32", dump, call);
      if (FILE *f = fopen(name, "wb"))
      {
        fwrite(kk.data(), 4, kk.size(), f);
        fclose(f);
      }
      snprintf(name, sizeof name, "%s.%d.goff.u64", dump, call);
      if (FILE *f = fopen(name, "wb"))
      {
        fwrite(go.data(), 8, go.size(), f);
        fclose(f);
      }
    }
    ++call;
  }
  std_sort_groups_tasks(key, idx, gof, goff, ng, n, b, st, chk ? key0 : nullptr);
}
void std_sort_info(uint64_t out[SORT_INFO_WORDS])
{
  const uint64_t c[SORT_INFO_WORDS] = {FIN_MAX, HEAP_BIG_MIN, HEAP_RANKED_MAX, HEAP_LARGE, SVC_WIDE_MIN, F2_HB, F2_EXT, HEAP_PAD, SJ_MAX_WIDE, SJ_MAX_NARROW,
                                       wide_lds_split(reinterpret_cast<const void *>(k_sort_job)).cap32};
  std::copy(c, c + SORT_INFO_WORDS, out);
}
static void window_sorts(uint32_t *key, uint32_t *idx, const uint32_t *gof, uint32_t n, hipStream_t st)
{
  hipLaunchKernelGGL(k_se_window_sort, dim3(cdiv(n, 256)), dim3(256), 0, st, key, idx, gof, n, 0u);
  if (n > 16) hipLaunchKernelGGL(k_se_window_sort, dim3(cdiv(n - 16, 256)), dim3(256), 0, st, key, idx, gof, n, 16u);
}
```

### breakid_amd/csrc/sortsvc.inc

```

constexpr uint32_t SVC_T_PART = 1, SVC_T_FIN = 2, SVC_T_HEAP = 3;
constexpr uint32_t SVC_WIDE_MIN = 16384;
constexpr uint32_t SVC_BIAS = 0x80000000u;
constexpr uint32_t SVC_MAX_JOBS = 64;
constexpr uint32_t SVC_H_QUIT = 0, SVC_H_ERROR = 1, SVC_H_NARROW = 8, SVC_H_STARTED = 16, SVC_H_DONE = SVC_H_STARTED + 1024, SVC_H_WORDS = SVC_H_DONE + SVC_MAX_JOBS;
constexpr uint32_t SVC_NARROW_LDS = 45056;
constexpr unsigned long long SVC_TIMEOUT_TICKS = 800000000ull;

struct SvcTask
{
  uint32_t type_job;
  uint32_t first, last;
  int32_t depth;
};
static_assert(sizeof(SvcTask) == 16, "two 8-byte halves");

struct SvcJob
{
  uint32_t *key, *idx, *posL, *posR;
  hent *hscratch;
  uint32_t *scratch32, *scratch32b;
  unsigned long long *rka, *rkb;
  uint32_t remaining;
  uint32_t done;
// ... 49 lines not shown
__device__ __forceinline__ void svc_release()
{
  __builtin_amdgcn_fence(__ATOMIC_RELEASE, "agent");
  asm volatile("s_waitcnt vmcnt(0)" ::: "memory");
}
__device__ __forceinline__ void svc_acquire()
{
  __builtin_amdgcn_fence(__ATOMIC_ACQUIRE, "agent");
  asm volatile("s_waitcnt vmcnt(0)" ::: "memory");
}

template <class T = WgTeam> __device__ __forceinline__ void svc_drain_barrier(const T &team = T())
{
  asm volatile("s_waitcnt vmcnt(0)" ::: "memory");
  team.sync();
}

__device__ __forceinline__ void svc_push(const SvcQueue &q, const SvcTask t, uint32_t *error)
{
  const uint32_t pos = atomicAdd(q.tail, 1u);
  const uint32_t slot = pos & q.mask;
  for (uint32_t spins = 0; svc_read(q.seq + slot) != pos; ++spins)
  {
    __builtin_amdgcn_s_sleep(16);
    if (spins > (1u << 22) || svc_read(error) != 0)
    {
      atomicOr(error, 2u);
      return;
    }
  }
  unsigned long long *d = reinterpret_cast<unsigned long long *>(q.slots + slot);
  svc_write(d, (unsigned long long) t.type_job | ((unsigned long long) t.first << 32));
  svc_write(d + 1, (unsigned long long) t.last | ((unsigned long long) (uint32_t) t.depth << 32));
  asm volatile("s_waitcnt vmcnt(0)" ::: "memory");
  svc_write(q.seq + slot, pos + 1u);
}
__device__ __forceinline__ uint32_t svc_ticket(const SvcQueue &q) { return atomicAdd(q.head, 1u); }
__device__ __forceinline__ bool svc_take(const SvcQueue &q, const uint32_t pos, SvcTask &t)
{
  const uint32_t slot = pos & q.mask;
  if (svc_read(q.seq + slot) != pos + 1u) return false;
  unsigned long long *s = reinterpret_cast<unsigned long long *>(q.slots + slot);
  const unsigned long long a = svc_read(s), b = svc_read(s + 1);
  t.type_job = (uint32_t) a;
  t.first = (uint32_t) (a >> 32);
  t.last = (uint32_t) b;
  t.depth = (int32_t) (uint32_t) (b >> 32);
  svc_write(q.seq + slot, pos + q.mask + 1u);
  return true;
}

__device__ __forceinline__ uint32_t svc_tag(uint32_t type, uint32_t job_tag) { return type | (job_tag << 4); }
__device__ __forceinline__ void svc_push_part(const SvcParams &P, uint32_t job_tag, uint32_t first, uint32_t last, int32_t depth)
{
  svc_push(P.q[(last - first) > SVC_WIDE_MIN ? 0 : 1], SvcTask{svc_tag(SVC_T_PART, job_tag), first, last, depth}, P.error);
}
__device__ __forceinline__ void svc_push_heap(const SvcParams &P, SvcJob *job, uint32_t job_tag, uint32_t first, uint32_t last)
{
  atomicMax(&job->max_heap, last - first);
  atomicAdd(&job->n_heap, last - first);
  svc_push(P.q[(last - first) > HEAP_BIG_MIN ? 0 : 1], SvcTask{svc_tag(SVC_T_HEAP, job_tag), first, last, 0}, P.error);
}
__device__ __forceinline__ void svc_done(const SvcParams &P, SvcJob *job, const uint32_t epoch)
{
  if (P.dbg) job->t_done = wall_clock64();
  svc_write(&job->done, 1u);
  __hip_atomic_store(P.host + SVC_H_DONE + (uint32_t) (job - P.jobs), epoch, __ATOMIC_RELAXED, __HIP_MEMORY_SCOPE_SYSTEM);
}
__device__ __forceinline__ void svc_retire(const SvcParams &P, SvcJob *job, const uint32_t job_tag, uint32_t dec)
{
  if (dec == 0) return;
  if (P.q[0].release & 2u) svc_release();
  if (atomicSub(&job->remaining, dec) == dec) svc_done(P, job, job_tag >> 8);
}

struct SvcJobLds
{
  uint32_t *key, *idx, *posL, *posR;
  hent *hscratch;
  uint32_t *scratch32, *scratch32b;
  unsigned long long *rka, *rkb;
  SvcJob *job;
  uint32_t tag;
};

__device__ __forceinline__ uint32_t svc_pick_pivot(uint32_t first, uint32_t last, uint32_t *key, uint32_t *idx)
{
  const uint32_t a = first + 1, b = first + (last - first) / 2, c = last - 1;
  const uint32_t ka = key[a], kb = key[b], kc = key[c];
  uint32_t pick;
  if (ka < kb)
  {
    if (kb < kc) pick = b;
    else if (ka < kc) pick = c;
    else pick = a;
  }
  else if (ka < kc) pick = a;
  else if (kb < kc) pick = c;
  else pick = b;
  const uint32_t kf = key[first], kp = key[pick];
  const uint32_t xf = idx[first], xp = idx[pick];
  st_through(key + first, kp);
  st_through(key + pick, kf);
  st_through(idx + first, xp);
  st_through(idx + pick, xf);
  return kp;
}

constexpr uint32_t TL_UNROLL = 24;
template <uint32_t NT> struct SvcPartLds
{
  uint32_t first, last, pivot;
  int32_t depth;
  uint32_t cnt[2][NT / 64];
  uint32_t cut;
  int go_on;
};
template <uint32_t NT, bool WIDE, class T = WgTeam>
__device__ __forceinline__ void svc_part(const SvcParams &P, const SvcJobLds &J, SvcPartLds<NT> &S, const SvcTask t, uint32_t *pos, const uint32_t pos_cap, const T &team = T())
{
  constexpr uint32_t NW = NT / 64;
  const uint32_t tid = team.tid(), lane = tid & 63, w = tid >> 6;
  uint32_t *key = J.key, *idx = J.idx;
  const uint32_t job_tag = t.type_job >> 4;
  uint32_t retired = 0;
  if (tid == 0)
  {
    S.first = t.first;
    S.last = t.last;
    S.go_on = 1;
    if (t.depth == 0)
    {
      svc_push_heap(P, J.job, job_tag, t.first, t.last);
      S.go_on = 0;
    }
    else if (t.last - t.first > pos_cap + 1u)
    {
      atomicOr(P.error, 32u);
      S.go_on = 0;
    }
    else
    {
      S.pivot = svc_pick_pivot(t.first, t.last, key, idx);
      S.depth = t.depth - 1;
      S.cut = 0xFFFFFFFFu;
    }
  }
  team.sync();
  if (!S.go_on) return;
  unsigned long long tph = 0;
  uint32_t *phase = (P.dbg && WIDE) ? P.dbg + 12 * 8192 + 32 : nullptr;
  auto mark = [&](int k) {
    if (phase && tid == 0)
    {
      const unsigned long long now = wall_clock64();
      if (k >= 0) atomicAdd(phase + k, (uint32_t) (now - tph));
      tph = now;
    }
  };
  for (;;)
  {
    const uint32_t first = S.first, last = S.last, pivot = S.pivot;
    const int32_t depth = S.depth;
    mark(-1);
    if (phase && tid == 0) atomicAdd(phase + 7, 1u);
    const uint32_t lo = first + 1, total = last - lo;
    const uint32_t chunk = (((total + NW - 1) / NW) + 63u) & ~63u;
    const uint32_t wbeg = lo + min(total, w * chunk), wend = lo + min(total, (w + 1) * chunk);
    uint32_t cL = 0, cR = 0;
    {
      uint32_t p = wbeg + lane;
      for (; p + (TL_UNROLL - 1) * 64 < wend; p += TL_UNROLL * 64)
      {
        uint32_t k[TL_UNROLL];
#pragma unroll
        for (uint32_t u = 0; u < TL_UNROLL; ++u) k[u] = key[p + u * 64];
#pragma unroll
        for (uint32_t u = 0; u < TL_UNROLL; ++u)
        {
          cL += k[u] >= pivot ? 1u : 0u;
          cR += k[u] <= pivot ? 1u : 0u;
        }
      }
      for (; p < wend; p += 64)
      {
        const uint32_t k = key[p];
        cL += k >= pivot ? 1u : 0u;
        cR += k <= pivot ? 1u : 0u;
      }
    }
    for (int d = 32; d >= 1; d >>= 1)
    {
      cL += __shfl_xor(cL, d, 64);
      cR += __shfl_xor(cR, d, 64);
    }
    if (lane == 0)
    {
      S.cnt[0][w] = cL;
      S.cnt[1][w] = cR;
    }
    team.sync();
    mark(0);
    uint32_t runL = 0, runR = 0, nL = 0, nR = 0;
    for (uint32_t i = 0; i < NW; ++i)
    {
      const uint32_t a = S.cnt[0][i], b = S.cnt[1][i];
      if (i < w)
      {
        runL += a;
        runR += b;
      }
      nL += a;
      nR += b;
    }
    uint32_t *pL = pos, *pR = pos + pos_cap;
    {
// ... 20 lines not shown
      {
        const uint32_t p = p0 + lane;
        const bool valid = p < wend;
        place(p, valid, valid ? key[p] : 0u);
      }
    }
    team.sync();
    mark(1);
    const uint32_t mm = nL < nR ? nL : nR;
    constexpr uint32_t SW = 4;
    for (uint32_t j0 = tid; j0 <= mm; j0 += SW * NT)
    {
      uint32_t lj[SW], rj[SW];
      bool sw[SW];
#pragma unroll
      for (uint32_t u = 0; u < SW; ++u)
      {
        const uint32_t j = j0 + u * NT;
        lj[u] = j < nL ? pL[j] : 0xFFFFFFFFu;
        rj[u] = j < nR ? pR[nR - 1 - j] : first;
      }
      uint32_t k1[SW], k2[SW], x1[SW], x2[SW];
#pragma unroll
      for (uint32_t u = 0; u < SW; ++u)
      {
        const uint32_t j = j0 + u * NT;
        sw[u] = j <= mm && (j < nL) && (j < nR) && (lj[u] < rj[u]);
        if (sw[u])
        {
          k1[u] = key[lj[u]];
          k2[u] = key[rj[u]];
          x1[u] = idx[lj[u]];
          x2[u] = idx[rj[u]];
        }
      }
#pragma unroll
      for (uint32_t u = 0; u < SW; ++u)
        if (sw[u])
        {
          st_through(key + lj[u], k2[u]);
          st_through(key + rj[u], k1[u]);
          st_through(idx + lj[u], x2[u]);
          st_through(idx + rj[u], x1[u]);
        }
#pragma unroll
      for (uint32_t u = 0; u < SW; ++u)
      {
        const uint32_t j = j0 + u * NT;
        if (j > mm || sw[u]) continue;
        const uint32_t ljj = lj[u];
        bool prev_cont = false;
        uint32_t rprev = 0;
        if (j > 0)
        {
          const uint32_t lp = pL[j - 1];
          rprev = pR[nR - j];
          prev_cont = lp < rprev;
        }
        if (j == 0)
          S.cut = ljj;
        else if (prev_cont)
          S.cut = ljj < rprev ? ljj : rprev;
      }
      if (!sw[SW - 1]) break;
    }
    svc_drain_barrier(team);
    mark(2);
    const uint32_t cut = S.cut;
    team.sync();
    if (cut == 0xFFFFFFFFu || cut <= first || cut > last)
    {
      if (tid == 0) SVC_FAIL(P, 8u, first, last, cut);
      return;
    }
    if (tid == 0)
    {
      const uint32_t a0 = first, a1 = cut, b0 = cut, b1 = last;
      const uint32_t sa = a1 - a0, sb = b1 - b0;
      const bool big_is_a = sa >= sb;
      const uint32_t g0 = big_is_a ? a0 : b0, g1 = big_is_a ? a1 : b1, h0 = big_is_a ? b0 : a0, h1 = big_is_a ? b1 : a1;
      const uint32_t sg = g1 - g0, sh = h1 - h0;
      const bool carry = sg > FIN_MAX && (!WIDE || sg > SVC_WIDE_MIN);
      const bool push_g = sg > 16 && !carry, push_h = sh > 16;
      retired += (sg <= 16 ? sg : 0u) + (sh <= 16 ? sh : 0u);
      const bool carry_heap = carry && depth == 0;
      if (push_g || push_h || carry_heap)
      {
        team.count_pushes((push_h ? 1u : 0u) + (push_g ? 1u : 0u));
        if (P.q[0].release & 1u) svc_release();
        if (push_h)
        {
          if (sh <= FIN_MAX)
            svc_push(P.q[1], SvcTask{svc_tag(SVC_T_FIN, job_tag), h0, h1, depth}, P.error);
          else
            svc_push_part(P, job_tag, h0, h1, depth);
        }
        if (push_g)
        {
          if (sg <= FIN_MAX)
            svc_push(P.q[1], SvcTask{svc_tag(SVC_T_FIN, job_tag), g0, g1, depth}, P.error);
          else
            svc_push_part(P, job_tag, g0, g1, depth);
        }
        if (carry_heap) svc_push_heap(P, J.job, job_tag, g0, g1);
      }
      if (carry && !carry_heap)
      {
        S.first = g0;
        S.last = g1;
        S.pivot = svc_pick_pivot(g0, g1, key, idx);
        S.depth = depth - 1;
        S.cut = 0xFFFFFFFFu;
        S.go_on = 1;
      }
      else
        S.go_on = 0;
    }
    svc_drain_barrier(team);
    mark(3);
    if (!S.go_on) break;
  }
  if (tid == 0 && retired) svc_retire(P, J.job, job_tag, retired);
}

constexpr uint32_t F2_HB = 256;
constexpr uint32_t F2_QCAP = 256;
constexpr uint32_t F2_EXT = 16;
struct Fin2Lds
{
  hent ent[FIN_MAX];
  uint16_t posL[FIN_MAX + 2], posR[FIN_MAX + 2];
  unsigned long long q[F2_QCAP];
  hent hbuf[4][F2_HB + 4];
  uint2 ext[F2_EXT];
  uint32_t q_head, q_tail, pending, n_ext, ext_elems, bad;
};
static_assert(sizeof(Fin2Lds) <= SVC_NARROW_LDS, "narrow workgroup LDS");
static_assert(FIN_MAX / F2_HB + 1 <= F2_EXT && FIN_MAX / 17 + 8 <= F2_QCAP, "fin2 lists");

__device__ __forceinline__ void f2_wsync()
{
  __builtin_amdgcn_fence(__ATOMIC_ACQ_REL, "wavefront");
  __builtin_amdgcn_wave_barrier();
}
__device__ __forceinline__ void f2_push(Fin2Lds &L, uint32_t first, uint32_t last, int32_t depth)
{
  const uint32_t slot = atomicAdd(&L.q_tail, 1u);
  if (slot >= F2_QCAP)
  {
    L.bad = 1u;
    return;
  }
  __hip_atomic_store(&L.q[slot], (unsigned long long) first | ((unsigned long long) last << 16) | ((unsigned long long) (uint32_t) (depth + 1) << 32), __ATOMIC_RELEASE, __HIP_MEMORY_SCOPE_WORKGROUP);
}
__device__ __forceinline__ uint32_t f2_partition(Fin2Lds &L, const uint32_t first, const uint32_t last, const uint32_t lane)
{
  hent *ent = L.ent;
  const uint32_t a = first + 1, b = first + (last - first) / 2, c = last - 1;
  const hent ea = ent[a], eb = ent[b], ec = ent[c];
  const uint32_t ka = hkey(ea), kb = hkey(eb), kc = hkey(ec);
  uint32_t pick;
  if (ka < kb)
  {
    if (kb < kc) pick = b;
    else if (ka < kc) pick = c;
    else pick = a;
  }
  else if (ka < kc) pick = a;
  else if (kb < kc) pick = c;
  else pick = b;
  const hent ep = pick == a ? ea : (pick == b ? eb : ec), ef = ent[first];
  const uint32_t pivot = hkey(ep);
  f2_wsync();
  if (lane == 0)
  {
    ent[first] = ep;
    ent[pick] = ef;
  }
  f2_wsync();
  uint16_t *pL = L.posL + first + 1, *pR = L.posR + first + 1;
  uint32_t nL = 0, nR = 0;
  for (uint32_t p0 = first + 1; p0 < last; p0 += 64)
  {
    const uint32_t p = p0 + lane;
    const bool valid = p < last;
    const uint32_t k = valid ? hkey(ent[p]) : 0u;
    const bool fL = valid && k >= pivot, fR = valid && k <= pivot;
    const unsigned long long mL = __ballot(fL), mR = __ballot(fR);
    if (fL) pL[nL + __builtin_amdgcn_mbcnt_hi((uint32_t) (mL >> 32), __builtin_amdgcn_mbcnt_lo((uint32_t) mL, 0u))] = (uint16_t) p;
// ... 82 lines not shown
      uint32_t retired = 0;
      bool go_on = false;
      if (depth == 0)
      {
        if (sz <= F2_HB)
        {
          hent *hb = L.hbuf[w];
          for (uint32_t i = lane; i < sz; i += 64) hb[i] = L.ent[first + i];
          f2_wsync();
          LdsMem mem{hb};
          make_heap_wave(mem, sz);
          sort_heap_asm<false>(hb, sz, 1);
          f2_wsync();
          for (uint32_t i = lane; i < sz; i += 64) L.ent[first + i] = hb[i];
          f2_wsync();
        }
        else if (lane == 0)
        {
          const uint32_t k = atomicAdd(&L.n_ext, 1u);
          if (k < F2_EXT) L.ext[k] = make_uint2(g0 + first, g0 + last); else L.bad = 1u;
          atomicAdd(&L.ext_elems, sz);
        }
        retired = sz;
      }
      else
      {
        const uint32_t cut = f2_partition(L, first, last, lane);
        if (cut <= first || cut > last)
        {
          if (lane == 0) L.bad = 2u;
          retired = sz;
        }
        else
        {
          const uint32_t sa = cut - first, sb = last - cut;
          const bool big_a = sa >= sb;
          const uint32_t h0 = big_a ? first : cut, h1 = big_a ? cut : last, l0 = big_a ? cut : first, l1 = big_a ? last : cut;
          const uint32_t sh = h1 - h0, sl = l1 - l0;
          --depth;
          if (sl > 16)
          {
            if (lane == 0) f2_push(L, l0, l1, depth);
          }
          else
            retired += sl;
          if (sh > 16)
          {
            first = h0;
            last = h1;
            go_on = true;
          }
          else
            retired += sh;
        }
      }
      if (retired && lane == 0) atomicSub(&L.pending, retired);
      if (!go_on) break;
    }
  }
  team.sync();
  for (uint32_t e = tid; e < m; e += 256)
  {
    const hent v = L.ent[e];
    st_through(key + g0 + e, hkey(v));
    st_through(idx + g0 + e, (uint32_t) v);
  }
}

static_assert((HEAP_BIG_MIN + HEAP_PAD) * 8 <= SVC_NARROW_LDS, "narrow workgroup LDS");

template <bool WIDE> __global__ __launch_bounds__(WIDE ? 1024 : 256) void k_sort_service(const SvcParams P)
{
  constexpr uint32_t NT = WIDE ? 1024u : 256u;
  extern __shared__ __attribute__((aligned(16))) unsigned char pool[];
  __shared__ SvcTask s_task;
  __shared__ int s_state;
  __shared__ SvcJobLds s_job;
  __shared__ SvcPartLds<NT> s_part;
  const uint32_t tid = threadIdx.x;
  const SvcQueue q = P.q[WIDE ? 0 : 1];
  if (tid == 0)
  {
    s_job.tag = 0xFFFFFFFFu;
    atomicAdd(P.stats + (WIDE ? 2 : 3), 1u);
    if (!WIDE && blockIdx.x == 0) __hip_atomic_store(P.host + SVC_H_NARROW, 1u, __ATOMIC_RELAXED, __HIP_MEMORY_SCOPE_SYSTEM);
    if (WIDE) __hip_atomic_store(P.host + SVC_H_STARTED + blockIdx.x, 1u, __ATOMIC_RELAXED, __HIP_MEMORY_SCOPE_SYSTEM);
  }
  unsigned long long t_last = wall_clock64();
  const unsigned long long t_start = t_last;
  uint32_t acc[8] = {0, 0, 0, 0, 0, 0, 0, 0};
  unsigned long long t_poll = t_last, t_task = t_last;
  for (;;)
  {
    if (tid == 0)
    {
      int st = 0;
      t_poll = wall_clock64();
      SvcTask t;
      uint32_t nap = 1, polls = 0;
      const uint32_t ticket = svc_ticket(q);
      uint32_t *dbg = P.dbg ? P.dbg + 4 * (blockIdx.x + (WIDE ? 0u : 4096u)) : nullptr;
      for (;;)
      {
        if (dbg)
        {
          SVC_ST(dbg, 1u);
          SVC_ST(dbg + 1, polls);
          SVC_ST(dbg + 2, (uint32_t) (wall_clock64() - t_start));
        }
        if (svc_take(q, ticket, t))
        {
          st = 1;
          break;
        }
        if (const uint32_t err = ((polls & 7u) == 0 ? svc_read(P.error) : 0u))
        {
          for (uint32_t k = 0; k < 4; ++k) __hip_atomic_store(P.host + SVC_H_ERROR + 1 + k, SVC_LD(P.error + 8 + k), __ATOMIC_RELAXED, __HIP_MEMORY_SCOPE_SYSTEM);
          __hip_atomic_store(P.host + SVC_H_ERROR, err, __ATOMIC_RELAXED, __HIP_MEMORY_SCOPE_SYSTEM);
          st = 2;
          if (dbg) SVC_ST(dbg + 3, 6u);
          break;
        }
        if ((++polls & 15u) == 0)
        {
          const uint32_t qv = svc_read(P.quit_d);
          if (qv == P.quit_word)
          {
            st = 2;
            if (dbg) SVC_ST(dbg + 3, 7u);
            break;
          }
          if (qv != 0u) atomicAdd(P.stats + 6, 1u);
        }
        if ((polls & 15u) == 0 && wall_clock64() - t_last > P.timeout_ticks)
        {
          atomicAdd(P.stats + (WIDE ? 4 : 5), 1u);
          st = 2;
          if (dbg) SVC_ST(dbg + 3, 8u);
          break;
        }
        for (uint32_t k = 0; k < nap; ++k) __builtin_amdgcn_s_sleep(32);
        if (nap < 4) ++nap;
      }
      if (st == 1)
      {
        svc_acquire();
        const uint32_t tag = t.type_job >> 4;
        if (s_job.tag != tag)
        {
          SvcJob *job = P.jobs + (tag & 0xFFu);
          unsigned long long *src = reinterpret_cast<unsigned long long *>(job);
          unsigned long long v[9];
#pragma unroll
          for (int k = 0; k < 9; ++k) v[k] = svc_read(src + k);
          s_job.key = (uint32_t *) v[0];
          s_job.idx = (uint32_t *) v[1];
          s_job.posL = (uint32_t *) v[2];
          s_job.posR = (uint32_t *) v[3];
          s_job.hscratch = (hent *) v[4];
          s_job.scratch32 = (uint32_t *) v[5];
          s_job.scratch32b = (uint32_t *) v[6];
          s_job.rka = (unsigned long long *) v[7];
          s_job.rkb = (unsigned long long *) v[8];
          s_job.job = job;
          s_job.tag = tag;
        }
// ... 205 lines not shown
      {
        asm volatile("s_waitcnt vmcnt(0)" ::: "memory");
        atomicSub(S.live, 1u);
      }
    }
    else if (type == SVC_T_HEAP)
    {
      const uint32_t m = t.last - t.first;
      if (WIDE)
        heap_big_body(t.first, t.last, J.key, J.idx, J.hscratch, J.scratch32, J.scratch32b, J.rka, J.rkb, reinterpret_cast<hent *>(pool), P.cap32, NT);
      else
        heap_small_body<T>(t.first, t.last, J.key, J.idx, reinterpret_cast<hent *>(pool), NT, team);
      svc_drain_barrier(team);
      if (tid == 0)
      {
        if (S.heavy && m > S.heavy_min) atomicMax(S.heavy + S.gof[t.first], m);
        if (S.trace)
        {
          const unsigned long long now = wall_clock64();
          atomicMax(S.trace + 1, ((unsigned long long) m << 40) | (t_task & 0xFFFFFFFFFFull));
          atomicMax(S.trace + 2, ((unsigned long long) m << 40) | ((now - t_task) & 0xFFFFFFFFFFull));
        }
        svc_retire(P, job, job_tag, m);
      }
    }
    else if (type == SVC_T_FIN && !WIDE)
    {
      Fin2Lds &L = *reinterpret_cast<Fin2Lds *>(pool);
      fin2_body<T>(L, t.first, t.last, t.depth, J.key, J.idx, team);
      svc_drain_barrier(team);
      if (tid == 0)
      {
        if (L.bad) SVC_FAIL(P, 64u, t.first, t.last, L.bad | (L.q_tail << 8) | (L.n_ext << 20));
        const uint32_t nh = L.n_ext < F2_EXT ? L.n_ext : F2_EXT;
        if (nh && (P.q[0].release & 1u)) svc_release();
        for (uint32_t k = 0; k < nh; ++k) svc_push_heap(P, job, job_tag, L.ext[k].x, L.ext[k].y);
        svc_retire(P, job, job_tag, (t.last - t.first) - L.ext_elems);
        asm volatile("s_waitcnt vmcnt(0)" ::: "memory");
        atomicSub(S.live, 1u);
      }
    }
    else if (tid == 0)
      SVC_FAIL(P, 16u, type, t.first, t.last);
    if (tid == 0)
    {
      t_last = wall_clock64();
      if (S.trace)
      {
        if (type != SVC_T_HEAP) atomicMax(S.trace + 3, t_last);
        atomicMax(S.trace + 4, t_last);
      }
    }
    team.sync();
  }
}

__global__ __launch_bounds__(1024) void k_sort_job(const SjParams S, const SvcJobLds J)
{
  extern __shared__ __attribute__((aligned(16))) unsigned char pool[];
  __shared__ SvcTask s_task[SJ_TEAMS];
  __shared__ int s_state[SJ_TEAMS];
  __shared__ uint32_t s_bar[SJ_TEAMS][2];
  __shared__ union
  {
    SvcPartLds<1024> wide;
    SvcPartLds<256> narrow[SJ_TEAMS];
  } s_part;
  if (blockIdx.x < S.n_wide)
  {
    sj_serve<true>(S, J, s_task[0], s_state[0], s_part.wide, pool, S.P.pos[0] + 2ull * S.P.pos_cap[0] * blockIdx.x, WgLive{{}, S.live});
    return;
  }
  const uint32_t team = threadIdx.x >> 8;
  if ((threadIdx.x & 255u) == 0)
  {
    s_bar[team][0] = 0u;
    s_bar[team][1] = 0u;
  }
  __syncthreads();
  sj_serve<false>(S, J, s_task[team], s_state[team], s_part.narrow[team], pool + team * SJ_TEAM_LDS,
                  S.P.pos[1] + 2ull * S.P.pos_cap[1] * ((blockIdx.x - S.n_wide) * SJ_TEAMS + team), LdsTeam{s_bar[team], team * 256u, S.live});
}

__global__ __launch_bounds__(256) void k_sort_job_submit(const SjParams S, const SvcJob desc, const uint64_t *__restrict__ goff, uint32_t ng)
{
  __shared__ uint32_t s_total, s_tasks;
  const SvcParams &P = S.P;
  SvcJob *job = P.jobs;
  const uint32_t job_tag = desc.epoch << 8;
  if (threadIdx.x == 0)
  {
    s_total = 0;
    s_tasks = 0;
    for (int k = 0; k < 2; ++k) svc_write(P.q[k].head, svc_read(P.q[k].tail));
    for (int k = 0; k < 12; ++k) svc_write(P.error + k, 0u);
    svc_write(S.live, 0u);
    if (S.trace)
    {
      svc_write(S.trace, ~0ull);
      for (int k = 1; k < 5; ++k) svc_write(S.trace + k, 0ull);
    }
    const unsigned long long *src = reinterpret_cast<const unsigned long long *>(&desc);
    unsigned long long *dst = reinterpret_cast<unsigned long long *>(job);
    for (uint32_t k = 0; k < sizeof(SvcJob) / 8; ++k)
      if (k != 9) svc_write(dst + k, src[k]);
    svc_write(&job->done, 0u);
    svc_write(&job->remaining, SVC_BIAS);
    asm volatile("s_waitcnt vmcnt(0)" ::: "memory");
    svc_release();
  }
  __syncthreads();
  uint32_t mine = 0, tasks = 0;
  for (uint32_t g = threadIdx.x; g < ng; g += blockDim.x)
  {
    const uint32_t first = (uint32_t) goff[g], last = (uint32_t) goff[g + 1], sz = last - first;
    if (sz <= 16) continue;
    mine += sz;
    ++tasks;
    const int32_t depth = 2 * (31 - __clz((int) sz));
    if (sz <= FIN_MAX)
      svc_push(P.q[1], SvcTask{svc_tag(SVC_T_FIN, job_tag), first, last, depth}, P.error);
    else
      svc_push_part(P, job_tag, first, last, depth);
  }
  atomicAdd(&s_total, mine);
  atomicAdd(&s_tasks, tasks);
  __syncthreads();
  if (threadIdx.x == 0)
  {
    svc_write(S.live, s_tasks);
    const uint32_t add = s_total - SVC_BIAS;
    if (atomicAdd(&job->remaining, add) + add == 0u) svc_done(P, job, desc.epoch);
  }
}
```

### include/breakid_hip.h

```cpp
#ifndef BREAKID_HIP_H
#define BREAKID_HIP_H

#include <stdint.h>
#include <stddef.h>

#ifdef __cplusplus
extern "C" {
#endif

#define BK_OK 0
#define BK_ERR_ARG (-1)
#define BK_ERR_HIP (-2)
#define BK_ERR_NO_DEVICE (-3)
#define BK_ERR_UNSORTED (-4)
#define BK_ERR_CIGAR (-5)
#define BK_ERR_IO (-6)
#define BK_ERR_LIMIT (-7)
#define BK_ERR_COLLISION (-8)

#define BK_MEM_HOST 0
#define BK_MEM_DEVICE 1

typedef struct bk_ctx bk_ctx;

// ... 274 lines not shown
#define BK_GAP_INS 1u
#define BK_GAP_MAX_TOL 100u
#define BK_GAP_MAX_LEN 1000000u
struct bk_cigar_gap {
  int32_t tid; uint32_t start; uint32_t len; uint32_t kind;
  uint32_t n_reads, n_rows, n_exact;
  uint32_t top_reads;
  uint32_t lo_start, hi_start, lo_len, hi_len;
  uint32_t n_fwd, n_rev;
  uint64_t mapq_sum;
};
int bk_cigar_gaps(bk_ctx *records, int mapq_min, uint32_t min_len, uint32_t anchor, uint32_t tol, uint32_t min_reads, const struct bk_cigar_gap **out, uint64_t *count);
int bk_cigar_gap_counts(bk_ctx *records, uint64_t out[8]);

#define BK_CLIP_LEFT 0u
#define BK_CLIP_RIGHT 1u
#define BK_CLIPLOCI_MAX_TOL 100u
#define BK_CLIPLOCI_MAX_PAIR 100000u
struct bk_clip_locus {
  int32_t tid; uint32_t pos; uint32_t dir;
  uint32_t flags;
  uint32_t n_reads, n_rows, n_exact;
  uint32_t top_reads;
  uint32_t lo_pos, hi_pos;
  uint32_t n_fwd, n_rev;
  uint32_t max_clip;
  uint32_t n_orphan;
  uint64_t clip_sum, mapq_sum;
  uint32_t n_improper;
  uint32_t claim;
  uint32_t mate;
  uint32_t mate_pos, mate_reads;
  int32_t mate_off;
};
int bk_clip_loci(bk_ctx *records, bk_ctx *calls, int mapq_min, int min_clip, uint32_t tol, uint32_t pair_dist, uint32_t min_reads, const struct bk_clip_locus **out,
                 uint64_t *count);
int bk_clip_locus_counts(bk_ctx *records, uint64_t out[8]);

int bk_fetch(bk_ctx *ctx, int stage, const void **data, uint64_t *count, const uint64_t **group_off, uint32_t *n_groups);

typedef struct bk_group_stat {
  int32_t p1_tid, p2_tid;
  uint64_t n_scan, n_isolated_removed, n_clustered;
  uint32_t cluster_id_end;
  uint32_t ordinal;
} bk_group_stat;
int bk_group_stats(bk_ctx *ctx, const bk_group_stat **out, uint32_t *n_groups);

int bk_timing(bk_ctx *ctx, const char *const **names, const float **ms, const uint64_t **bytes, int *n);
int bk_timing_enable(bk_ctx *ctx, int on);
int bk_timing_touched(bk_ctx *ctx, const uint64_t **touched, int *n);

typedef struct bk_shard_stats {
  uint64_t isize_sum, isize_n;
  double sumsq;
  uint32_t vmax, max_span;
  uint64_t n_cand, n_split;
} bk_shard_stats;
#define BK_BUF_CANDIDATES 0
#define BK_BUF_TUPLES 1
#define BK_BUF_CLUSTERS 2
int bk_shard_begin(bk_ctx *ctx, uint64_t rec_base, int mapq_min);
int bk_shard_get_stats(bk_ctx *ctx, bk_shard_stats *out);
int bk_shard_set_stats(bk_ctx *ctx, const bk_shard_stats *total);
int bk_shard_sd_local(bk_ctx *ctx, uint64_t *l_total, void **ex_dev, uint64_t *n_ex);
int bk_shard_sd_finish(bk_ctx *ctx, const void *all_ex_dev, uint64_t n_all, uint64_t l_grand, double *mean, double *sd);
int bk_shard_buffer(bk_ctx *ctx, int which, void **dev, uint64_t *count, uint32_t *elem_bytes);
int bk_shard_set_buffer(bk_ctx *ctx, int which, const void *dev, uint64_t count);
int bk_shard_group_sizes(bk_ctx *ctx, const uint64_t **starts, uint32_t *n_groups);
int bk_shard_own_groups(bk_ctx *ctx, const uint8_t *own, uint32_t n_groups);
int bk_shard_route_candidates(bk_ctx *ctx, uint32_t world, void **dev, const uint64_t **counts);
int bk_shard_group_keys(bk_ctx *ctx, const uint32_t **keys, uint32_t *n_groups);
int bk_shard_route_pairs(bk_ctx *ctx, const uint32_t *dest_of_group, uint32_t n_groups, uint32_t world, void **dev, const uint64_t **counts);
int bk_shard_group_pairs(bk_ctx *ctx, const void *pairs_dev, uint64_t n, const uint32_t *all_keys, uint32_t n_all_keys);
int bk_shard_bp_cov(bk_ctx *ctx, double w, void **cov_dev, uint64_t *n);
int bk_shard_bp_vote(bk_ctx *ctx, double w, const void *cov_total_dev);
int bk_shard_bp_vote_slice(bk_ctx *ctx, double w, const void *cov_total_dev, uint64_t lo, uint64_t hi, void **clusters_dev, void **voted_dev);
int bk_shard_bp_set_voted(bk_ctx *ctx, const void *voted_all_dev);
int bk_shard_bp_depth(bk_ctx *ctx, void **depth_dev, uint64_t *n);
int bk_shard_bp_finish(bk_ctx *ctx, const void *depth_total_dev);

int bk_debug_std_sort(bk_ctx *ctx, const uint32_t *key, const uint64_t *group_off, uint32_t n_groups, uint32_t *perm_out);

int bk_debug_scan(bk_ctx *ctx, int elem_bytes, const void *in, uint64_t n, int in_place, void *out);
int bk_debug_radix_sort(bk_ctx *ctx, const uint64_t *keys, const uint32_t *vals, uint64_t n, int begin_bit, int end_bit, uint64_t *keys_out, uint32_t *vals_out);
int bk_debug_prims_info(uint64_t out[4]);

int bk_sort_forms(bk_ctx *ctx, uint64_t out[3]);

int bk_debug_sort_info(bk_ctx *ctx, uint64_t out[13]);

int bk_debug_ahc(bk_ctx *ctx, const uint32_t *x, const uint32_t *y, uint32_t n, double w, uint32_t *idx_out, int32_t *cluster_out, uint32_t *n_out);

int bk_debug_points(bk_ctx *ctx, int mode, const uint32_t *x, const uint32_t *y, uint32_t n, double w, uint32_t *idx_out, int32_t *cluster_out, uint32_t *n_out);
int bk_debug_points_groups(bk_ctx *ctx, int mode, const uint32_t *x, const uint32_t *y, const uint64_t *group_off, uint32_t n_groups, double w, uint32_t *idx_out,
                           int32_t *cluster_out, uint64_t *goff_out, uint32_t *n_out);
int bk_debug_cluster_info(uint64_t out[2]);
int bk_debug_stream_info(uint64_t out[4]);
int bk_debug_stream_blocks(unsigned blocks);
int bk_debug_cigar(bk_ctx *ctx, uint32_t n, const uint8_t *kind, const uint32_t *c1_off, const uint8_t *c1, const uint32_t *c2_off, const uint8_t *c2, const int32_t *e,
                   int32_t *out6);
int bk_debug_vote(bk_ctx *ctx, const bk_split *side1, uint32_t n1, const bk_split *side2, uint32_t n2, int32_t p1_tid, int32_t p2_tid, int32_t *out3);
int bk_debug_region(bk_ctx *ctx, int32_t tid, uint32_t start, uint32_t end, uint64_t depth_pos, bk_split *out, uint32_t cap, uint32_t *n_out, uint32_t *cov_out,
                    uint32_t *depth_out);

typedef struct bk_bam bk_bam;
uint64_t bk_qname_hash(const char *name, size_t len);
uint32_t bk_qname_check(const char *name, size_t len);
int bk_bam_open(const char *path, bk_bam **out, char *err, size_t errlen);
int bk_bam_header(const bk_bam *b, int *n_targets, const char *const **names, const uint32_t **lens);
int bk_bam_decode(bk_bam *b, bk_soa *out, char *err, size_t errlen);
void bk_bam_close(bk_bam *b);
typedef struct bk_read_key { uint64_t qhash; uint32_t qcheck; uint32_t tag; } bk_read_key;
int bk_bam_extract(const char *in_bam, const char *out_bam, const bk_read_key *keys, uint64_t n_keys, const char *const *tags, uint64_t n_tags, char **names_out,
                   uint64_t *n_written, char *err, size_t errlen);
void bk_bam_names_free(char *names);
int bk_bam_reads(const char *in_bam, const bk_read_key *keys, uint64_t n_keys, bk_reads *out, char *err, size_t errlen);
void bk_reads_free(bk_reads *r);

typedef struct bk_bam_dev bk_bam_dev;
int bk_bam_decode_device(const char *path, int device, bk_bam_dev **out, bk_soa *cols, int *n_targets, const char *const **names, const uint32_t **lens,
                         char *err, size_t errlen);
int bk_bam_decode_device_part(const char *path, int device, int part, int parts, bk_bam_dev **out, bk_soa *cols, int *n_targets, const char *const **names,
                              const uint32_t **lens, char *err, size_t errlen);
void bk_bam_dev_free(bk_bam_dev *h);
void bk_feed_release_caches(void);
int bk_bam_decode_device_ctx(const char *path, int device, int mapq_min, bk_bam_dev **bam_out, bk_ctx **ctx_out, int *n_targets, const char *const **names,
                             const uint32_t **lens, char *err, size_t errlen);
int bk_records(bk_ctx *ctx, bk_soa *cols);
int bk_debug_bgzf_inflate(const void *file, uint64_t n, void *out, uint64_t out_cap, uint64_t *out_len, float *kernel_ms, char *err, size_t errlen);

#ifdef __cplusplus
}
#endif
#endif
```

Baseline: 11750.

## Defer large heap-sort segments and overlap their finish with lane replanning

During the observed mask pass, the sort service now defers large depth-exhausted segments above a threshold (default 28672, env-tunable) instead of heap-sorting them inline. It copies them aside and finishes them in a separate job on the lane stream. The host waits only on an event marking the list's readiness, replans lanes while deferred sorts continue, and pins groups with pending heaps to their lane, adding the pending heap cost to the lane cost model. This is meant to take the long tail of heavy heap sorts off the critical path between phases, at the cost of extra copies, event and stream coordination complexity, and a bounded defer buffer.

```diff
diff --git a/breakid_amd/capi.py b/breakid_amd/capi.py
--- a/breakid_amd/capi.py
+++ b/breakid_amd/capi.py
@@ -30,7 +30,7 @@
 EXPORTS = ["bk_init", "bk_prepare_process", "bk_free", "bk_last_error", "bk_set_stream", "bk_sync", "bk_get_stream", "bk_upload_records", "bk_records", "bk_exclude_regions", "bk_isize_stats",
            "bk_discordant_pairs", "bk_mask_and_cluster", "bk_split_evidence", "bk_cluster_summary",
            "bk_split_breakpoints", "bk_normal_support", "bk_ref_support", "bk_genotype_call", "bk_clip_support", "bk_clip_reads", "bk_base_depth", "bk_clip_rescue", "bk_junctions", "bk_junction_sides", "bk_vcf_breakend_alt", "bk_evidence", "bk_unique_support", "bk_clip_consensus", "bk_junction_fit", "bk_locus_similarity", "bk_site_complexity", "bk_window_coverage", "bk_window_context", "bk_call_windows", "bk_fusion_frame", "bk_link_calls", "bk_locus_partners", "bk_call_partner_sites", "bk_fragment_sizes", "bk_fragment_bounds", "bk_known_calls", "bk_split_junctions", "bk_split_junction_counts", "bk_debug_split_junctions", "bk_cigar_gaps", "bk_cigar_gap_counts", "bk_clip_loci", "bk_clip_locus_counts", "bk_run", "bk_fetch", "bk_timing", "bk_timing_enable", "bk_timing_touched", "bk_group_stats", "bk_qname_hash", "bk_qname_check",
-           "bk_bam_open", "bk_bam_header", "bk_bam_decode", "bk_bam_close", "bk_bam_extract", "bk_bam_names_free", "bk_bam_reads", "bk_reads_free", "bk_bam_decode_device", "bk_bam_decode_device_part", "bk_bam_decode_device_ctx", "bk_bam_dev_free", "bk_feed_release_caches", "bk_debug_bgzf_inflate", "bk_debug_std_sort", "bk_debug_scan", "bk_debug_radix_sort", "bk_debug_prims_info", "bk_sort_forms", "bk_debug_sort_info", "bk_debug_ahc", "bk_debug_points", "bk_debug_points_groups", "bk_debug_cluster_info", "bk_debug_stream_info", "bk_debug_stream_blocks", "bk_debug_cigar", "bk_debug_vote", "bk_debug_region", "bk_shard_begin", "bk_shard_get_stats", "bk_shard_set_stats",
+           "bk_bam_open", "bk_bam_header", "bk_bam_decode", "bk_bam_close", "bk_bam_extract", "bk_bam_names_free", "bk_bam_reads", "bk_reads_free", "bk_bam_decode_device", "bk_bam_decode_device_part", "bk_bam_decode_device_ctx", "bk_bam_dev_free", "bk_feed_release_caches", "bk_debug_bgzf_inflate", "bk_debug_std_sort", "bk_debug_defer_sort", "bk_debug_scan", "bk_debug_radix_sort", "bk_debug_prims_info", "bk_sort_forms", "bk_debug_sort_info", "bk_debug_ahc", "bk_debug_points", "bk_debug_points_groups", "bk_debug_cluster_info", "bk_debug_stream_info", "bk_debug_stream_blocks", "bk_debug_cigar", "bk_debug_vote", "bk_debug_region", "bk_shard_begin", "bk_shard_get_stats", "bk_shard_set_stats",
            "bk_shard_sd_local", "bk_shard_sd_finish", "bk_shard_buffer", "bk_shard_set_buffer", "bk_shard_group_sizes",
            "bk_shard_own_groups", "bk_shard_route_candidates", "bk_shard_group_keys", "bk_shard_route_pairs", "bk_shard_group_pairs", "bk_shard_bp_cov", "bk_shard_bp_vote", "bk_shard_bp_vote_slice", "bk_shard_bp_set_voted", "bk_shard_bp_depth", "bk_shard_bp_finish"]
 
@@ -102,6 +102,7 @@
         L.bk_timing_enable.argtypes = [vp, C.c_int]
         L.bk_timing_touched.argtypes = [vp, C.POINTER(C.POINTER(C.c_uint64)), C.POINTER(C.c_int)]
         L.bk_debug_std_sort.argtypes = [vp, vp, vp, C.c_uint32, vp]
+        L.bk_debug_defer_sort.argtypes = [vp, vp, vp, C.c_uint32, C.c_uint32, C.c_uint32, vp, vp, u64p]
         L.bk_debug_scan.argtypes = [vp, C.c_int, vp, C.c_uint64, C.c_int, vp]
         L.bk_debug_radix_sort.argtypes = [vp, vp, vp, C.c_uint64, C.c_int, C.c_int, vp, vp]
         L.bk_debug_prims_info.argtypes = [u64p]
@@ -738,6 +739,17 @@
         self._check(self.L.bk_debug_std_sort(self.h, key.ctypes.data, group_off.ctypes.data, len(group_off) - 1, perm.ctypes.data))
         return perm
 
+    DEFER_INFO = ("deferred", "beyond_cap", "longest", "elements", "stage_deferred", "stage_pinned")
+
+    def debug_defer_sort(self, key, group_off, defer_min, defer_cap=0):
+        key = np.ascontiguousarray(key, np.uint32)
+        group_off = np.ascontiguousarray(group_off, np.uint64)
+        perm, kout = np.zeros(len(key), np.uint32), np.zeros(len(key), np.uint32)
+        out = (C.c_uint64 * len(self.DEFER_INFO))()
+        self._check(self.L.bk_debug_defer_sort(self.h, key.ctypes.data, group_off.ctypes.data, len(group_off) - 1, int(defer_min), int(defer_cap),
+                                               perm.ctypes.data, kout.ctypes.data, out))
+        return perm, kout, dict(zip(self.DEFER_INFO, (int(v) for v in out)))
+
     def debug_scan(self, values, in_place=False):
         values = np.ascontiguousarray(values)
         assert values.ndim == 1 and values.dtype in (np.uint32, np.uint64), values.dtype
diff --git a/breakid_amd/csrc/api.hip b/breakid_amd/csrc/api.hip
--- a/breakid_amd/csrc/api.hip
+++ b/breakid_amd/csrc/api.hip
@@ -2454,6 +2454,29 @@
   });
 }
 
+int bk_debug_defer_sort(bk_ctx *ctx, const uint32_t *key, const uint64_t *group_off, uint32_t n_groups, uint32_t defer_min, uint32_t defer_cap, uint32_t *perm_out, uint32_t *key_out, uint64_t out[6])
+{
+  return guarded(ctx, [&] {
+    if (!key || !group_off || !perm_out || !key_out || !out) throw bk_error(BK_ERR_ARG, "bk_debug_defer_sort: null argument");
+    const uint64_t n = group_off[n_groups];
+    DevBuf dk, dp, dgof, dgoff;
+    std::vector<uint32_t> gof(n), iota(n);
+    for (uint32_t g = 0; g < n_groups; ++g)
+      for (uint64_t p = group_off[g]; p < group_off[g + 1]; ++p) gof[p] = g;
+    std::iota(iota.begin(), iota.end(), 0u);
+    HIP_CHECK(hipMemcpy(dk.as<uint32_t>(n + 1), key, n * 4, hipMemcpyHostToDevice));
+    HIP_CHECK(hipMemcpy(dp.as<uint32_t>(n + 1), iota.data(), n * 4, hipMemcpyHostToDevice));
+    HIP_CHECK(hipMemcpy(dgof.as<uint32_t>(n + 1), gof.data(), n * 4, hipMemcpyHostToDevice));
+    HIP_CHECK(hipMemcpy(dgoff.as<uint64_t>((uint64_t) n_groups + 1), group_off, ((uint64_t) n_groups + 1) * 8, hipMemcpyHostToDevice));
+    ctx->stage.debug_defer_sort(ctx->st, dk.get<uint32_t>(), dp.get<uint32_t>(), dgof.get<uint32_t>(), dgoff.get<uint64_t>(), n_groups, n, defer_min, defer_cap, out);
+    out[4] = ctx->stage.defer_stats[0];
+    out[5] = ctx->stage.defer_stats[1];
+    HIP_CHECK(hipMemcpyAsync(perm_out, dp.get<uint32_t>(), n * 4, hipMemcpyDeviceToHost, ctx->st));
+    HIP_CHECK(hipMemcpyAsync(key_out, dk.get<uint32_t>(), n * 4, hipMemcpyDeviceToHost, ctx->st));
+    HIP_CHECK(hipStreamSynchronize(ctx->st));
+  });
+}
+
 int bk_debug_scan(bk_ctx *ctx, int elem_bytes, const void *in, uint64_t n, int in_place, void *out)
 {
   return guarded(ctx, [&] {
diff --git a/breakid_amd/csrc/cluster.h b/breakid_amd/csrc/cluster.h
--- a/breakid_amd/csrc/cluster.h
+++ b/breakid_amd/csrc/cluster.h
@@ -21,6 +21,7 @@
 {
   std::vector<uint32_t> heavy_x, heavy_y;
   bool observe = false;
+  uint32_t defer_min = 0;
   uint64_t max_group_bound = 0;
   DevBuf key, perm, tmp, cnt, off, off2, idx2, gof2, goff2, jump, mark, apos, kid, kprev2, k1, k2, pk, knum, clfull, small, scan_tmp;
   SortEmuBufs se;
diff --git a/breakid_amd/csrc/cluster.hip b/breakid_amd/csrc/cluster.hip
--- a/breakid_amd/csrc/cluster.hip
+++ b/breakid_amd/csrc/cluster.hip
@@ -312,8 +312,22 @@
 
 void remove_isolated_end(const bk_pair *pairs, PairList &L, ClusterBufs &b, hipStream_t st)
 {
+  b.se.deferred.clear();
   if (L.n == 0 || L.ng == 0) return;
-  sort_list(pairs, L, 0, nullptr, 0, b, st);
+  b.se.defer_min = b.defer_min;
+  b.se.defer_src = b.defer_min ? L.idx.get<uint32_t>() : nullptr;
+  try
+  {
+    sort_list(pairs, L, 0, nullptr, 0, b, st);
+  }
+  catch (...)
+  {
+    b.se.defer_min = 0;
+    b.se.defer_src = nullptr;
+    throw;
+  }
+  b.se.defer_min = 0;
+  b.se.defer_src = nullptr;
 }
 
 namespace
diff --git a/breakid_amd/csrc/lanes.h b/breakid_amd/csrc/lanes.h
--- a/breakid_amd/csrc/lanes.h
+++ b/breakid_amd/csrc/lanes.h
@@ -30,8 +30,11 @@
     PairList list, iso;
     DevBuf d_cluster;
     hipStream_t st = nullptr;
+    hipEvent_t ev_list = nullptr, ev_fin = nullptr;
     ~Lane()
     {
+      if (ev_list) (void) hipEventDestroy(ev_list);
+      if (ev_fin) (void) hipEventDestroy(ev_fin);
       if (st) (void) hipStreamDestroy(st);
     }
   };
@@ -43,9 +46,11 @@
   uint64_t iso_n = 0;
   PairList lane_mid, lane_iso_m;
   DevBuf d_drop;
+  uint64_t defer_stats[2] = {0, 0};
 
   ClusterStage() { lanes.emplace_back(new Lane()); }
   void run(const StageInput &in, double w, int fast);
   void sort_forms(uint64_t out[3]) const;
+  void debug_defer_sort(hipStream_t st, uint32_t *key, uint32_t *idx, const uint32_t *gof, const uint64_t *goff, uint32_t ng, uint64_t n, uint32_t defer_min, uint32_t defer_cap, uint64_t stats[4]);
   void debug_sort(int device, hipStream_t st, uint32_t *key, uint32_t *idx, const uint32_t *gof, const uint64_t *goff, uint32_t ng, uint64_t n, uint64_t max_group);
 };
diff --git a/breakid_amd/csrc/lanes.hip b/breakid_amd/csrc/lanes.hip
--- a/breakid_amd/csrc/lanes.hip
+++ b/breakid_amd/csrc/lanes.hip
@@ -28,6 +28,11 @@
   if (svc) return want_svc < 1 ? 1 : (want_svc > 26 ? 26 : want_svc);
   static const int want = env ? atoi(env) : std::min(4, stage_queues());
   return want < 1 ? 1 : (want > 26 ? 26 : want);
+}
+static uint32_t lanes_defer_min()
+{
+  static const uint32_t v = getenv("BREAKID_DEFER_MIN") ? (uint32_t) strtoul(getenv("BREAKID_DEFER_MIN"), nullptr, 10) : 28672u;
+  return v;
 }
 static bool lanes_apply(const StageInput &in, int fast)
 {
@@ -284,7 +289,8 @@
   }
   return p;
 }
-static LanePlan plan_observed(const std::vector<uint64_t> &sizes, const std::vector<uint32_t> &hx, const std::vector<uint32_t> &hy, int K)
+static LanePlan plan_observed(const std::vector<uint64_t> &sizes, const std::vector<uint32_t> &hx, const std::vector<uint32_t> &hy, int K, const std::vector<int> &pin,
+                              const std::vector<uint32_t> &pend)
 {
   const uint32_t ng = (uint32_t) sizes.size();
   constexpr double per_pair = 0.001;
@@ -298,14 +304,26 @@
   });
   LanePlan p(ng, 0);
   std::vector<double> mx(K, 0.0), my(K, 0.0), pairs(K, 0.0);
-  auto cost = [&](int l) { return mx[l] + my[l] + per_pair * pairs[l]; };
+  std::vector<double> pre(K, 0.0);
+  for (int l = 0; l < K; ++l) pre[l] = heap_cost(pend[l]);
+  auto cost = [&](int l) { return pre[l] + mx[l] + my[l] + per_pair * pairs[l]; };
   for (uint32_t g : order)
   {
+    if (pin[g] < 0) continue;
+    const int l = pin[g];
+    mx[l] = std::max(mx[l], heap_cost(hx[g]));
+    my[l] = std::max(my[l], heap_cost(hy[g]));
+    pairs[l] += (double) sizes[g];
+    p[g] = l;
+  }
+  for (uint32_t g : order)
+  {
+    if (pin[g] >= 0) continue;
     int best = 0;
     double best_cost = 0;
     for (int l = 0; l < K; ++l)
     {
-      const double c = std::max(mx[l], heap_cost(hx[g])) + std::max(my[l], heap_cost(hy[g])) + per_pair * (pairs[l] + (double) sizes[g]);
+      const double c = pre[l] + std::max(mx[l], heap_cost(hx[g])) + std::max(my[l], heap_cost(hy[g])) + per_pair * (pairs[l] + (double) sizes[g]);
       if (l == 0 || c < best_cost || (c == best_cost && cost(l) < cost(best)))
       {
         best = l;
@@ -320,9 +338,12 @@
   if (bk_debug("lanes"))
     for (int l = 0; l < K; ++l)
     {
-      fprintf(stderr, "[lanes] lane %d: max heap x %.0f y %.0f, %.0f pairs, cost %.0f; heavy groups:", l, mx[l], my[l], pairs[l], cost(l));
+      fprintf(stderr, "[lanes] lane %d: max heap x %.0f y %.0f, %.0f pairs, pending heap %u, cost %.0f; heavy groups:", l, mx[l], my[l], pairs[l], pend[l], cost(l));
       for (uint32_t g = 0; g < ng; ++g)
         if (p[g] == l && (hx[g] || hy[g])) fprintf(stderr, " %u(%u,%u)", g, hx[g], hy[g]);
+      fprintf(stderr, "; pinned groups:");
+      for (uint32_t g = 0; g < ng; ++g)
+        if (pin[g] == l) fprintf(stderr, " %u", g);
       fprintf(stderr, "\n");
     }
   return p;
@@ -382,12 +403,13 @@
   uint32_t *drop_base = nullptr;
   auto lane_drop = [&](int l) { return drop_base + (size_t) l * ((size_t) ng + 1); };
   std::vector<std::vector<uint8_t>> keep(K, std::vector<uint8_t>(ng, 0));
-  auto upload_plan = [&](const LanePlan &p) {
+  auto upload_plan = [&](const LanePlan &p, hipStream_t st) {
     for (int l = 0; l < K; ++l)
       for (uint32_t g = 0; g < ng; ++g) keep[l][g] = p[g] == l ? 1 : 0;
-    drop_base = upload_drop(p, K, cs.d_drop, in.st);
-  };
-  auto in_lanes = [&](auto body) {
+    drop_base = upload_drop(p, K, cs.d_drop, st);
+  };
+  auto stream_through = [&](int l) { HIP_CHECK(hipStreamSynchronize(lane_st(l))); };
+  auto in_lanes = [&](auto body, auto settle) {
     std::vector<std::string> err(K);
     std::vector<int> code(K, BK_OK);
     const auto t_start = std::chrono::steady_clock::now();
@@ -395,7 +417,7 @@
       try
       {
         body(l);
-        HIP_CHECK(hipStreamSynchronize(lane_st(l)));
+        settle(l);
         if (dbg)
           fprintf(stderr, "[lanes] lane %d done after %.2f ms\n", l, std::chrono::duration<double, std::milli>(std::chrono::steady_clock::now() - t_start).count());
       }
@@ -414,9 +436,13 @@
     guarded_body(0);
     for (std::thread &t : th) t.join();
     for (int l = 0; l < K; ++l)
-      if (code[l] != BK_OK) throw bk_error(code[l], err[l]);
-  };
-  auto merge_all = [&](PairList ClusterStage::Lane::*which, PairList &out, DevBuf *cl_out) {
+      if (code[l] != BK_OK)
+      {
+        for (int k = 0; k < K; ++k) (void) hipStreamSynchronize(lane_st(k));
+        throw bk_error(code[l], err[l]);
+      }
+  };
+  auto merge_all = [&](PairList ClusterStage::Lane::*which, PairList &out, DevBuf *cl_out, hipStream_t st) {
     std::vector<const PairList *> ls(K);
     std::vector<const uint32_t *> cls(K);
     for (int l = 0; l < K; ++l)
@@ -424,7 +450,7 @@
       ls[l] = &(lane(l).*which);
       cls[l] = lane(l).d_cluster.get<uint32_t>();
     }
-    merge_lists_many(ls.data(), cl_out ? cls.data() : nullptr, K, out, cl_out, in.st);
+    merge_lists_many(ls.data(), cl_out ? cls.data() : nullptr, K, out, cl_out, st);
   };
   const bk_pair *pairs = in.jr.pairs;
   auto mask_lane = [&](int l, bool observe) {
@@ -438,7 +464,9 @@
     }
     remove_isolated_begin(pairs, in.jr.gof, in.jr.gstart, ng, in.jr.n_pairs, w, lane(l).list, cb, lane_st(l), lane_drop(l), in.gstart_host.data(), keep[l].data());
     if (observe) cb.heavy_x.assign(ng, 0u);
+    cb.defer_min = observe ? lanes_defer_min() : 0u;
     remove_isolated_end(pairs, lane(l).list, cb, lane_st(l));
+    cb.defer_min = 0;
     if (observe) cb.observe = false;
   };
   auto cluster_lane = [&](int l) {
@@ -452,21 +480,42 @@
   auto phase = [&](const char *what) {
     if (dbg) fprintf(stderr, "[lanes] %s at %.2f ms\n", what, std::chrono::duration<double, std::milli>(std::chrono::steady_clock::now() - tp0).count());
   };
-  upload_plan(plan_blind(in, K));
+  upload_plan(plan_blind(in, K), in.st);
   phase("plan uploaded");
+  cs.defer_stats[0] = cs.defer_stats[1] = 0;
   if (use_svc)
     in_lanes([&](int l) {
       mask_lane(l, false);
       cluster_lane(l);
-    });
+    }, stream_through);
   else
   {
-    in_lanes([&](int l) { mask_lane(l, true); });
+    for (int l = 0; l < K; ++l)
+      for (hipEvent_t *e : {&lane(l).ev_list, &lane(l).ev_fin})
+        if (!*e) HIP_CHECK(hipEventCreate(e));
+    in_lanes(
+        [&](int l) {
+          mask_lane(l, true);
+          HIP_CHECK(hipEventRecord(lane(l).ev_list, lane_st(l)));
+          std_sort_finish_deferred(lane(l).cb.se, lane_st(l));
+          HIP_CHECK(hipEventRecord(lane(l).ev_fin, lane_st(l)));
+        },
+        [&](int l) { HIP_CHECK(hipEventSynchronize(lane(l).ev_list)); });
+    auto fin_done = [&](int l) {
+      const hipError_t e = hipEventQuery(lane(l).ev_fin);
+      if (e != hipSuccess && e != hipErrorNotReady) throw bk_error(BK_ERR_HIP, std::string("lanes: finish job: ") + hipGetErrorString(e));
+      return e == hipSuccess;
+    };
+    int bl = -1;
+    while (bl < 0)
+      for (int l = 0; l < K && bl < 0; ++l)
+        if (fin_done(l)) bl = l;
+    const hipStream_t bst = lane_st(bl);
     PairList &mid = cs.lane_mid;
-    merge_all(&ClusterStage::Lane::list, mid, nullptr);
+    merge_all(&ClusterStage::Lane::list, mid, nullptr, bst);
     std::vector<uint64_t> goff_h((size_t) ng + 1);
-    HIP_CHECK(hipMemcpyAsync(goff_h.data(), mid.goff.get<uint64_t>(), ((size_t) ng + 1) * 8, hipMemcpyDeviceToHost, in.st));
-    HIP_CHECK(hipStreamSynchronize(in.st));
+    HIP_CHECK(hipMemcpyAsync(goff_h.data(), mid.goff.get<uint64_t>(), ((size_t) ng + 1) * 8, hipMemcpyDeviceToHost, bst));
+    HIP_CHECK(hipStreamSynchronize(bst));
     std::vector<uint64_t> sizes(ng);
     std::vector<uint32_t> hx(ng, 0u), hy(ng, 0u);
     for (uint32_t g = 0; g < ng; ++g) sizes[g] = goff_h[g + 1] - goff_h[g];
@@ -476,19 +525,64 @@
         hx[g] = std::max(hx[g], lane(l).cb.heavy_x[g]);
         hy[g] = std::max(hy[g], lane(l).cb.heavy_y[g]);
       }
-    upload_plan(plan_observed(sizes, hx, hy, K));
-    in_lanes([&](int l) {
-      list_subset_ranges(mid, goff_h.data(), keep[l].data(), lane(l).list, lane_st(l));
-      cluster_lane(l);
-    });
+    std::vector<int> pin(ng, -1);
+    std::vector<uint32_t> pend(K, 0u);
+    for (int l = 0; l < K; ++l)
+    {
+      const auto &df = lane(l).cb.se.deferred;
+      cs.defer_stats[0] += df.size();
+      if (df.empty() || fin_done(l)) continue;
+      for (const auto &d : df)
+      {
+        if (d.group < ng && pin[d.group] < 0) ++cs.defer_stats[1];
+        if (d.group < ng) pin[d.group] = l;
+        pend[l] = std::max(pend[l], d.last - d.first);
+      }
+    }
+    upload_plan(plan_observed(sizes, hx, hy, K, pin, pend), bst);
+    phase("second plan uploaded");
+    in_lanes(
+        [&](int l) {
+          PairList &L = lane(l).list;
+          list_subset_ranges(mid, goff_h.data(), keep[l].data(), L, lane_st(l));
+          uint64_t at = 0;
+          std::vector<uint64_t> dgoff(ng);
+          for (uint32_t g = 0; g < ng; ++g)
+          {
+            dgoff[g] = at;
+            at += keep[l][g] ? sizes[g] : 0;
+          }
+          for (int o = 0; o < K; ++o)
+            for (const auto &d : lane(o).cb.se.deferred)
+              if (d.group < ng && keep[l][d.group])
+              {
+                const uint64_t to = dgoff[d.group] + (d.first - d.group_first);
+                if (to + (d.last - d.first) > L.n) throw bk_error(BK_ERR_HIP, "lanes: a deferred segment outside its group");
+                std_sort_scatter_deferred(lane(o).cb.se, d, L.idx.get<uint32_t>() + to, nullptr, lane_st(l));
+              }
+          cluster_lane(l);
+          std_sort_finish_check(lane(l).cb.se, lane_st(l));
+        },
+        stream_through);
+    if (dbg)
+      for (int l = 0; l < K; ++l)
+      {
+        const auto &df = lane(l).cb.se.deferred;
+        if (df.empty()) continue;
+        float ms = 0;
+        uint32_t longest = 0;
+        for (const auto &d : df) longest = std::max(longest, d.last - d.first);
+        (void) hipEventElapsedTime(&ms, lane(l).ev_list, lane(l).ev_fin);
+        fprintf(stderr, "[lanes] lane %d finish job: %zu segments deferred, the longest %u elements; ended %.2f ms after the lane reported%s\n", l, df.size(), longest, ms, pend[l] ? " (groups pinned)" : "");
+      }
   }
   phase("lanes done");
   svc_stage.finish();
   phase("service stopped");
   if (use_svc && bk_debug("lanes")) fprintf(stderr, "[svc] tasks: %u wide, %u narrow\n", cs.svc.stats[0], cs.svc.stats[1]);
   PairList &iso_m = cs.lane_iso_m;
-  merge_all(&ClusterStage::Lane::iso, iso_m, nullptr);
-  merge_all(&ClusterStage::Lane::list, cs.list, &cs.d_cluster);
+  merge_all(&ClusterStage::Lane::iso, iso_m, nullptr, in.st);
+  merge_all(&ClusterStage::Lane::list, cs.list, &cs.d_cluster, in.st);
   HIP_CHECK(hipStreamSynchronize(in.st));
   phase("lists merged");
   cs.iso_n = iso_m.n;
@@ -531,3 +625,38 @@
   std_sort_groups(key, idx, gof, goff, ng, n, cb().se, st);
   svc_stage.finish();
 }
+
+void ClusterStage::debug_defer_sort(hipStream_t st, uint32_t *key, uint32_t *idx, const uint32_t *gof, const uint64_t *goff, uint32_t ng, uint64_t n, uint32_t defer_min, uint32_t defer_cap, uint64_t stats[4])
+{
+  SortEmuBufs &se = cb().se;
+  const uint32_t cap0 = se.defer_cap;
+  se.deferred.clear();
+  se.df_beyond_cap = 0;
+  se.defer_min = defer_min;
+  se.defer_cap = defer_cap ? defer_cap : cap0;
+  se.defer_src = nullptr;
+  try
+  {
+    std_sort_groups(key, idx, gof, goff, ng, n, se, st);
+  }
+  catch (...)
+  {
+    se.defer_min = 0;
+    se.defer_cap = cap0;
+    throw;
+  }
+  se.defer_min = 0;
+  se.defer_cap = cap0;
+  std_sort_finish_deferred(se, st);
+  stats[0] = se.deferred.size();
+  stats[1] = se.df_beyond_cap;
+  stats[2] = stats[3] = 0;
+  for (const auto &d : se.deferred)
+  {
+    std_sort_scatter_deferred(se, d, idx + d.first, key + d.first, st);
+    stats[2] = std::max<uint64_t>(stats[2], d.last - d.first);
+    stats[3] += d.last - d.first;
+  }
+  std_sort_finish_check(se, st);
+  HIP_CHECK(hipStreamSynchronize(st));
+}
diff --git a/breakid_amd/csrc/sortemu.h b/breakid_amd/csrc/sortemu.h
--- a/breakid_amd/csrc/sortemu.h
+++ b/breakid_amd/csrc/sortemu.h
@@ -39,6 +39,21 @@
   bool tj_ready = false;
   uint64_t sorts[2] = {0, 0};
   uint32_t last_heap[2] = {0, 0};
+  struct Deferred
+  {
+    uint32_t first, last;
+    uint32_t off;
+    uint32_t group, group_first;
+  };
+  uint32_t defer_min = 0, defer_cap = 64;
+  const uint32_t *defer_src = nullptr;
+  DevBuf df_list, df_off, df_key, df_idx, df_err;
+  std::vector<Deferred> deferred;
+  uint32_t df_beyond_cap = 0;
+  uint32_t df_n = 0;
+  uint32_t df_cap = 0;
+  uint64_t df_max_group = 0;
+  bool df_unchecked = false;
   SortEmuBufs() = default;
   SortEmuBufs(const SortEmuBufs &) = delete;
   SortEmuBufs &operator=(const SortEmuBufs &) = delete;
@@ -46,5 +61,9 @@
 
 void std_sort_groups(uint32_t *key, uint32_t *idx, const uint32_t *gof, const uint64_t *goff, uint32_t ng, uint64_t n, SortEmuBufs &b, hipStream_t st);
 
+void std_sort_finish_deferred(SortEmuBufs &b, hipStream_t st);
+void std_sort_finish_check(SortEmuBufs &b, hipStream_t st);
+void std_sort_scatter_deferred(const SortEmuBufs &b, const SortEmuBufs::Deferred &d, uint32_t *dst_idx, uint32_t *dst_key, hipStream_t st);
+
 constexpr int SORT_INFO_WORDS = 11;
 void std_sort_info(uint64_t out[SORT_INFO_WORDS]);
diff --git a/breakid_amd/csrc/sortemu.hip b/breakid_amd/csrc/sortemu.hip
--- a/breakid_amd/csrc/sortemu.hip
+++ b/breakid_amd/csrc/sortemu.hip
@@ -1128,7 +1128,56 @@
   window_sorts(key, idx, gof, n, st);
 }
 
-static void std_sort_groups_tasks(uint32_t *key, uint32_t *idx, const uint32_t *gof, const uint64_t *goff, uint32_t ng, uint32_t n, SortEmuBufs &b, hipStream_t st, const uint32_t *key0)
+static SjParams sj_setup(SortEmuBufs &b, uint32_t n, uint64_t max_group, uint32_t n_wide, uint32_t n_narrow, uint32_t cap32, hipStream_t st)
+{
+  SjParams S = {};
+  SvcParams &P = S.P;
+  auto pow2 = [](uint64_t v) {
+    uint32_t c = 1024;
+    while (c < v && c < (1u << 30)) c <<= 1;
+    return c;
+  };
+  const uint32_t want[2] = {pow2((uint64_t) n / HEAP_BIG_MIN + 4096), pow2((uint64_t) n / 16 + 4096)};
+  for (int k = 0; k < 2; ++k)
+    if (want[k] > b.tj_cap[k])
+    {
+      b.tj_cap[k] = want[k];
+      b.tj_ready = false;
+    }
+  uint32_t *ctl = b.tj_ctl.as<uint32_t>(SJ_C_WORDS);
+  for (int k = 0; k < 2; ++k)
+  {
+    P.q[k].head = ctl + 64 * k;
+    P.q[k].tail = ctl + 64 * k + 32;
+    P.q[k].slots = b.tj_slots[k].as<SvcTask>(b.tj_cap[k]);
+    P.q[k].seq = b.tj_seq[k].as<uint32_t>(b.tj_cap[k]);
+    P.q[k].mask = b.tj_cap[k] - 1;
+    P.q[k].release = 1u;
+  }
+  P.error = ctl + SJ_C_ERROR;
+  P.stats = ctl + SJ_C_STATS;
+  P.quit_d = ctl + SJ_C_QUIT;
+  P.host = ctl + SJ_C_HOST;
+  P.jobs = b.tj_jobs.as<SvcJob>(SVC_MAX_JOBS);
+  P.cap32 = cap32;
+  P.quit_word = 0u;
+  P.timeout_ticks = SJ_TIMEOUT_TICKS;
+  P.pos_cap[0] = (uint32_t) std::max<uint64_t>(max_group, SVC_WIDE_MIN) + 64;
+  P.pos_cap[1] = SVC_WIDE_MIN + 64;
+  P.pos[0] = b.tj_pos[0].as<uint32_t>(2ull * P.pos_cap[0] * n_wide);
+  P.pos[1] = b.tj_pos[1].as<uint32_t>(2ull * P.pos_cap[1] * n_narrow * SJ_TEAMS);
+  P.dbg = nullptr;
+  S.n_wide = n_wide;
+  S.live = ctl + SJ_C_LIVE;
+  if (!b.tj_ready)
+  {
+    HIP_CHECK(hipMemsetAsync(b.tj_ctl.p, 0, SJ_C_WORDS * 4, st));
+    hipLaunchKernelGGL(k_svc_reset, dim3(cdiv(std::max(b.tj_cap[0], b.tj_cap[1]), 256)), dim3(256), 0, st, P);
+    b.tj_ready = true;
+  }
+  return S;
+}
+static void sj_kernel_lds(size_t &dyn_lds_out, uint32_t &cap32_out)
 {
   static size_t dyn_lds = 0;
   static uint32_t cap32 = 0;
@@ -1140,6 +1189,22 @@
     if (dyn_lds < SJ_TEAMS * SJ_TEAM_LDS) throw bk_error(BK_ERR_HIP, "k_sort_job: the narrow teams do not fit the LDS");
     HIP_CHECK(hipFuncSetAttribute(reinterpret_cast<const void *>(k_sort_job), hipFuncAttributeMaxDynamicSharedMemorySize, (int) dyn_lds));
   });
+  dyn_lds_out = dyn_lds;
+  cap32_out = cap32;
+}
+
+static void finish_job_verdict(const uint32_t fe[13], SortEmuBufs &b)
+{
+  if (fe[0] == 0u && fe[12] == 0u) return;
+  b.tj_ready = false;
+  throw bk_error(fe[0] & 2u ? BK_ERR_LIMIT : BK_ERR_HIP, "sort task dispatch: the job of the deferred heaps: task error " + std::to_string(fe[0]) + ", " + std::to_string(fe[12]) + " elements not final; first failing task: code " + std::to_string(fe[8]) + ", " + std::to_string(fe[9]) + " " + std::to_string(fe[10]) + " " + std::to_string(fe[11]));
+}
+
+static void std_sort_groups_tasks(uint32_t *key, uint32_t *idx, const uint32_t *gof, const uint64_t *goff, uint32_t ng, uint32_t n, SortEmuBufs &b, hipStream_t st, const uint32_t *key0)
+{
+  size_t dyn_lds = 0;
+  uint32_t cap32 = 0;
+  sj_kernel_lds(dyn_lds, cap32);
   std::vector<uint64_t> go((size_t) ng + 1);
   HIP_CHECK(hipMemcpyAsync(go.data(), goff, go.size() * 8, hipMemcpyDeviceToHost, st));
   HIP_CHECK(hipStreamSynchronize(st));
@@ -1147,62 +1212,31 @@
   for (uint32_t g = 0; g < ng; ++g) max_group = std::max<uint64_t>(max_group, go[g + 1] - go[g]);
   const uint32_t n_wide = std::min<uint32_t>(SJ_MAX_WIDE, std::max<uint32_t>(1, cdiv(n, 1u << 16)));
   const uint32_t n_narrow = std::min<uint32_t>(SJ_MAX_NARROW, std::max<uint32_t>(1, cdiv(n, 1u << 16)));
-  SjParams S = {};
+  SjParams S = sj_setup(b, n, max_group, n_wide, n_narrow, cap32, st);
   SvcParams &P = S.P;
-  {
-    auto pow2 = [](uint64_t v) {
-      uint32_t c = 1024;
-      while (c < v && c < (1u << 30)) c <<= 1;
-      return c;
-    };
-    const uint32_t want[2] = {pow2((uint64_t) n / HEAP_BIG_MIN + 4096), pow2((uint64_t) n / 16 + 4096)};
-    for (int k = 0; k < 2; ++k)
-      if (want[k] > b.tj_cap[k])
-      {
-        b.tj_cap[k] = want[k];
-        b.tj_ready = false;
-      }
-    uint32_t *ctl = b.tj_ctl.as<uint32_t>(SJ_C_WORDS);
-    for (int k = 0; k < 2; ++k)
-    {
-      P.q[k].head = ctl + 64 * k;
-      P.q[k].tail = ctl + 64 * k + 32;
-      P.q[k].slots = b.tj_slots[k].as<SvcTask>(b.tj_cap[k]);
-      P.q[k].seq = b.tj_seq[k].as<uint32_t>(b.tj_cap[k]);
-      P.q[k].mask = b.tj_cap[k] - 1;
-      P.q[k].release = 1u;
-    }
-    P.error = ctl + SJ_C_ERROR;
-    P.stats = ctl + SJ_C_STATS;
-    P.quit_d = ctl + SJ_C_QUIT;
-    P.host = ctl + SJ_C_HOST;
-    P.jobs = b.tj_jobs.as<SvcJob>(SVC_MAX_JOBS);
-    P.cap32 = cap32;
-    P.quit_word = 0u;
-    P.timeout_ticks = SJ_TIMEOUT_TICKS;
-    P.pos_cap[0] = (uint32_t) std::max<uint64_t>(max_group, SVC_WIDE_MIN) + 64;
-    P.pos_cap[1] = SVC_WIDE_MIN + 64;
-    P.pos[0] = b.tj_pos[0].as<uint32_t>(2ull * P.pos_cap[0] * n_wide);
-    P.pos[1] = b.tj_pos[1].as<uint32_t>(2ull * P.pos_cap[1] * n_narrow * SJ_TEAMS);
-    P.dbg = nullptr;
-    S.n_wide = n_wide;
-    S.live = ctl + SJ_C_LIVE;
-    S.gof = gof;
-    S.heavy_min = b.heavy_all ? FIN_MAX : HEAP_RANKED_MIN;
-    if (b.heavy)
-    {
-      S.heavy = b.tj_heavy.as<uint32_t>(ng);
-      HIP_CHECK(hipMemsetAsync(S.heavy, 0, (size_t) ng * 4, st));
-    }
+  S.gof = gof;
+  S.heavy_min = b.heavy_all ? FIN_MAX : HEAP_RANKED_MIN;
+  if (b.heavy)
+  {
+    S.heavy = b.tj_heavy.as<uint32_t>(ng);
+    HIP_CHECK(hipMemsetAsync(S.heavy, 0, (size_t) ng * 4, st));
+  }
+  const uint32_t defer_cap = b.defer_min ? std::max<uint32_t>(1, b.defer_cap) : 0u;
+  uint32_t *defer = nullptr, *soff = nullptr, *skey = nullptr, *sidx = nullptr;
+  if (b.defer_min)
+  {
+    defer = b.df_list.as<uint32_t>(2 + 2ull * defer_cap);
+    soff = b.df_off.as<uint32_t>(defer_cap);
+    skey = b.df_key.as<uint32_t>((uint64_t) n + HEAP_PAD);
+    sidx = b.df_idx.as<uint32_t>((uint64_t) n + HEAP_PAD);
+    b.deferred.clear();
+    b.df_beyond_cap = 0;
+    b.df_n = n;
+    b.df_cap = defer_cap;
+    b.df_max_group = max_group;
   }
   static const bool dbg = bk_debug("svc");
   if (dbg) S.trace = b.tj_trace.as<unsigned long long>(8);
-  if (!b.tj_ready)
-  {
-    HIP_CHECK(hipMemsetAsync(b.tj_ctl.p, 0, SJ_C_WORDS * 4, st));
-    hipLaunchKernelGGL(k_svc_reset, dim3(cdiv(std::max(b.tj_cap[0], b.tj_cap[1]), 256)), dim3(256), 0, st, P);
-    b.tj_ready = true;
-  }
   SvcJob d = {};
   d.key = key;
   d.idx = idx;
@@ -1212,15 +1246,26 @@
   d.rka = b.rk_a.as<unsigned long long>((uint64_t) n + HEAP_PAD);
   d.rkb = b.rk_b.as<unsigned long long>((uint64_t) n + HEAP_PAD);
   d.epoch = (b.tj_epoch++ % 0xFFFFFu) + 1u;
-  const SvcJobLds J = {d.key, d.idx, nullptr, nullptr, d.hscratch, d.scratch32, d.scratch32b, d.rka, d.rkb, P.jobs, d.epoch << 8};
-  hipLaunchKernelGGL(k_sort_job_submit, dim3(1), dim3(256), 0, st, S, d, goff, ng);
+  const SvcJobLds J = {d.key, d.idx, nullptr, nullptr, d.hscratch, d.scratch32, d.scratch32b, d.rka, d.rkb, P.jobs, d.epoch << 8, defer, b.defer_min, defer_cap};
+  hipLaunchKernelGGL(k_sort_job_submit, dim3(1), dim3(256), 0, st, S, d, goff, ng, defer);
   hipLaunchKernelGGL(k_sort_job, dim3(n_wide + n_narrow), dim3(1024), dyn_lds, st, S, J);
   HIP_CHECK(hipGetLastError());
   ++b.sorts[1];
-  if (key0) sort_check("after the task dispatch", key, idx, key0, n, goff, ng, st, b);
+  if (key0 && !defer) sort_check("after the task dispatch", key, idx, key0, n, goff, ng, st, b);
+  if (defer)
+    hipLaunchKernelGGL(k_defer_copy, dim3(defer_cap), dim3(256), 0, st, defer, defer_cap, key, idx, b.defer_src, n, skey, sidx, soff, S.heavy, gof, S.heavy_min);
   window_sorts(key, idx, gof, n, st);
   uint32_t h[16] = {};
   HIP_CHECK(hipMemcpyAsync(h, P.error, 12 * 4, hipMemcpyDeviceToHost, st));
+  std::vector<uint32_t> dl;
+  if (defer)
+  {
+    dl.resize(2 + 2 * (size_t) defer_cap);
+    HIP_CHECK(hipMemcpyAsync(dl.data(), defer, dl.size() * 4, hipMemcpyDeviceToHost, st));
+  }
+  uint32_t fe[16] = {};
+  const bool fin_look = b.df_unchecked;
+  if (fin_look) HIP_CHECK(hipMemcpyAsync(fe, b.df_err.as<uint32_t>(16), 13 * 4, hipMemcpyDeviceToHost, st));
   std::vector<uint32_t> hv;
   if (S.heavy)
   {
@@ -1234,6 +1279,11 @@
   HIP_CHECK(hipStreamSynchronize(st));
   b.last_heap[0] = j.max_heap;
   b.last_heap[1] = j.n_heap;
+  if (fin_look)
+  {
+    b.df_unchecked = false;
+    finish_job_verdict(fe, b);
+  }
   if (h[0] || j.remaining != 0u)
   {
     b.tj_ready = false;
@@ -1244,8 +1294,23 @@
     if (b.heavy->size() < ng) b.heavy->resize(ng, 0u);
     for (uint32_t g = 0; g < ng; ++g) (*b.heavy)[g] = std::max((*b.heavy)[g], hv[g]);
   }
+  if (defer)
+  {
+    const uint32_t cnt = std::min(dl[0], defer_cap);
+    b.df_beyond_cap = dl[0] - cnt;
+    uint32_t off = 0;
+    for (uint32_t k = 0; k < cnt; ++k)
+    {
+      const uint32_t first = dl[2 + 2 * k], last = dl[3 + 2 * k];
+      if (first >= last || last > n || off + (last - first) > n) throw bk_error(BK_ERR_HIP, "sort task dispatch: a deferred segment outside the array");
+      const uint32_t g = (uint32_t) (std::upper_bound(go.begin(), go.end(), (uint64_t) first) - go.begin()) - 1;
+      b.deferred.push_back({first, last, off, g, (uint32_t) go[g]});
+      off += last - first;
+    }
+  }
   if (S.trace)
   {
+    if (defer) fprintf(stderr, "[svc] task dispatch %u: %zu heap segments deferred (more than %u elements each), %u more found the list full\n", d.epoch, b.deferred.size(), b.defer_min, b.df_beyond_cap);
     const double t0 = (double) tr[0];
     const uint32_t hm = (uint32_t) (tr[1] >> 40);
     const unsigned long long hs = tr[1] & 0xFFFFFFFFFFull, base = tr[0] & ~0xFFFFFFFFFFull;
@@ -1254,6 +1319,52 @@
     fprintf(stderr, "[svc] task dispatch %u: %u elements in %u groups on %u wide + %u narrow workgroups; longest heap %u elements started %.3f ms after the dispatch and took %.3f ms; partitions and finisher done after %.3f ms, job after %.3f ms; %u elements in heaps, the longest %u\n",
             d.epoch, n, ng, n_wide, n_narrow, hm, hm ? ((double) hstart - t0) * 1e-5 : 0.0, hm ? (double) (tr[2] & 0xFFFFFFFFFFull) * 1e-5 : 0.0, tr[3] ? ((double) tr[3] - t0) * 1e-5 : 0.0, ((double) tr[4] - t0) * 1e-5, j.n_heap, j.max_heap);
   }
+}
+
+void std_sort_finish_deferred(SortEmuBufs &b, hipStream_t st)
+{
+  if (b.deferred.empty()) return;
+  size_t dyn_lds = 0;
+  uint32_t cap32 = 0;
+  sj_kernel_lds(dyn_lds, cap32);
+  uint32_t big = 0, small = 0;
+  for (const SortEmuBufs::Deferred &d : b.deferred) ++((d.last - d.first) > HEAP_BIG_MIN ? big : small);
+  const uint32_t n = b.df_n, n_wide = std::min<uint32_t>(SJ_MAX_WIDE, std::max<uint32_t>(1, big)), n_narrow = std::min<uint32_t>(SJ_MAX_NARROW, std::max<uint32_t>(1, cdiv(small, SJ_TEAMS)));
+  SjParams S = sj_setup(b, n, b.df_max_group, n_wide, n_narrow, cap32, st);
+  SvcParams &P = S.P;
+  static const bool dbg = bk_debug("svc");
+  if (dbg) S.trace = b.tj_trace.as<unsigned long long>(8);
+  SvcJob d = {};
+  d.key = b.df_key.get<uint32_t>();
+  d.idx = b.df_idx.get<uint32_t>();
+  d.hscratch = b.heap_scratch.as<hent>((uint64_t) n + HEAP_PAD);
+  d.scratch32 = b.scratch32.as<uint32_t>((uint64_t) n + HEAP_PAD);
+  d.scratch32b = b.scratch32b.as<uint32_t>((uint64_t) n + HEAP_PAD);
+  d.rka = b.rk_a.as<unsigned long long>((uint64_t) n + HEAP_PAD);
+  d.rkb = b.rk_b.as<unsigned long long>((uint64_t) n + HEAP_PAD);
+  d.epoch = (b.tj_epoch++ % 0xFFFFFu) + 1u;
+  const SvcJobLds J = {d.key, d.idx, nullptr, nullptr, d.hscratch, d.scratch32, d.scratch32b, d.rka, d.rkb, P.jobs, d.epoch << 8, nullptr, 0u, 0u};
+  const uint32_t cap = b.df_cap;
+  hipLaunchKernelGGL(k_sort_job_submit_heaps, dim3(1), dim3(256), 0, st, S, d, b.df_list.get<uint32_t>(), cap, b.df_off.get<uint32_t>());
+  hipLaunchKernelGGL(k_sort_job, dim3(n_wide + n_narrow), dim3(1024), dyn_lds, st, S, J);
+  hipLaunchKernelGGL(k_sort_job_stash, dim3(1), dim3(64), 0, st, P.error, P.jobs, b.df_err.as<uint32_t>(16));
+  HIP_CHECK(hipGetLastError());
+  b.df_unchecked = true;
+}
+void std_sort_finish_check(SortEmuBufs &b, hipStream_t st)
+{
+  if (!b.df_unchecked) return;
+  uint32_t fe[16] = {};
+  HIP_CHECK(hipMemcpyAsync(fe, b.df_err.as<uint32_t>(16), 13 * 4, hipMemcpyDeviceToHost, st));
+  HIP_CHECK(hipStreamSynchronize(st));
+  b.df_unchecked = false;
+  finish_job_verdict(fe, b);
+}
+void std_sort_scatter_deferred(const SortEmuBufs &b, const SortEmuBufs::Deferred &d, uint32_t *dst_idx, uint32_t *dst_key, hipStream_t st)
+{
+  const uint32_t m = d.last - d.first;
+  hipLaunchKernelGGL(k_copy_u32, dim3(cdiv(m, 256)), dim3(256), 0, st, b.df_idx.get<uint32_t>() + d.off, dst_idx, m);
+  if (dst_key) hipLaunchKernelGGL(k_copy_u32, dim3(cdiv(m, 256)), dim3(256), 0, st, b.df_key.get<uint32_t>() + d.off, dst_key, m);
 }
 
 void std_sort_groups(uint32_t *key, uint32_t *idx, const uint32_t *gof, const uint64_t *goff, uint32_t ng, uint64_t n64, SortEmuBufs &b, hipStream_t st)
diff --git a/breakid_amd/csrc/sortsvc.inc b/breakid_amd/csrc/sortsvc.inc
--- a/breakid_amd/csrc/sortsvc.inc
+++ b/breakid_amd/csrc/sortsvc.inc
@@ -155,7 +155,21 @@
   unsigned long long *rka, *rkb;
   SvcJob *job;
   uint32_t tag;
+  uint32_t *defer;
+  uint32_t defer_min, defer_cap;
 };
+
+__device__ __forceinline__ bool svc_defer_heap(const SvcJobLds &J, uint32_t first, uint32_t last)
+{
+  if (!J.defer || last - first <= J.defer_min) return false;
+  const uint32_t k = atomicAdd(J.defer, 1u);
+  if (k >= J.defer_cap) return false;
+  J.defer[2 + 2 * k] = first;
+  J.defer[3 + 2 * k] = last;
+  atomicMax(&J.job->max_heap, last - first);
+  atomicAdd(&J.job->n_heap, last - first);
+  return true;
+}
 
 __device__ __forceinline__ uint32_t svc_pick_pivot(uint32_t first, uint32_t last, uint32_t *key, uint32_t *idx)
 {
@@ -204,7 +218,10 @@
     S.go_on = 1;
     if (t.depth == 0)
     {
-      svc_push_heap(P, J.job, job_tag, t.first, t.last);
+      if (svc_defer_heap(J, t.first, t.last))
+        svc_retire(P, J.job, job_tag, t.last - t.first);
+      else
+        svc_push_heap(P, J.job, job_tag, t.first, t.last);
       S.go_on = 0;
     }
     else if (t.last - t.first > pos_cap + 1u)
@@ -391,8 +408,16 @@
       const uint32_t sg = g1 - g0, sh = h1 - h0;
       const bool carry = sg > FIN_MAX && (!WIDE || sg > SVC_WIDE_MIN);
       const bool push_g = sg > 16 && !carry, push_h = sh > 16;
+      bool carry_deferred = false;
       retired += (sg <= 16 ? sg : 0u) + (sh <= 16 ? sh : 0u);
-      const bool carry_heap = carry && depth == 0;
+      bool carry_heap = carry && depth == 0;
+      if (carry_heap && svc_defer_heap(J, g0, g1))
+      {
+        retired += sg;
+        carry_heap = false;
+        S.go_on = 0;
+        carry_deferred = true;
+      }
       if (push_g || push_h || carry_heap)
       {
         team.count_pushes((push_h ? 1u : 0u) + (push_g ? 1u : 0u));
@@ -413,7 +438,7 @@
         }
         if (carry_heap) svc_push_heap(P, J.job, job_tag, g0, g1);
       }
-      if (carry && !carry_heap)
+      if (carry && !carry_heap && !carry_deferred)
       {
         S.first = g0;
         S.last = g1;
@@ -662,6 +687,7 @@
   if (tid == 0)
   {
     s_job.tag = 0xFFFFFFFFu;
+    s_job.defer = nullptr;
     atomicAdd(P.stats + (WIDE ? 2 : 3), 1u);
     if (!WIDE && blockIdx.x == 0) __hip_atomic_store(P.host + SVC_H_NARROW, 1u, __ATOMIC_RELAXED, __HIP_MEMORY_SCOPE_SYSTEM);
     if (WIDE) __hip_atomic_store(P.host + SVC_H_STARTED + blockIdx.x, 1u, __ATOMIC_RELAXED, __HIP_MEMORY_SCOPE_SYSTEM);
@@ -1033,7 +1059,29 @@
                   S.P.pos[1] + 2ull * S.P.pos_cap[1] * ((blockIdx.x - S.n_wide) * SJ_TEAMS + team), LdsTeam{s_bar[team], team * 256u, S.live});
 }
 
-__global__ __launch_bounds__(256) void k_sort_job_submit(const SjParams S, const SvcJob desc, const uint64_t *__restrict__ goff, uint32_t ng)
+__device__ __forceinline__ void sj_submit_begin(const SjParams &S, const SvcJob &desc, uint32_t *defer)
+{
+  const SvcParams &P = S.P;
+  SvcJob *job = P.jobs;
+  if (defer) svc_write(defer, 0u);
+  for (int k = 0; k < 2; ++k) svc_write(P.q[k].head, svc_read(P.q[k].tail));
+  for (int k = 0; k < 12; ++k) svc_write(P.error + k, 0u);
+  svc_write(S.live, 0u);
+  if (S.trace)
+  {
+    svc_write(S.trace, ~0ull);
+    for (int k = 1; k < 5; ++k) svc_write(S.trace + k, 0ull);
+  }
+  const unsigned long long *src = reinterpret_cast<const unsigned long long *>(&desc);
+  unsigned long long *dst = reinterpret_cast<unsigned long long *>(job);
+  for (uint32_t k = 0; k < sizeof(SvcJob) / 8; ++k)
+    if (k != 9) svc_write(dst + k, src[k]);
+  svc_write(&job->done, 0u);
+  svc_write(&job->remaining, SVC_BIAS);
+  asm volatile("s_waitcnt vmcnt(0)" ::: "memory");
+  svc_release();
+}
+__global__ __launch_bounds__(256) void k_sort_job_submit(const SjParams S, const SvcJob desc, const uint64_t *__restrict__ goff, uint32_t ng, uint32_t *defer)
 {
   __shared__ uint32_t s_total, s_tasks;
   const SvcParams &P = S.P;
@@ -1043,22 +1091,7 @@
   {
     s_total = 0;
     s_tasks = 0;
-    for (int k = 0; k < 2; ++k) svc_write(P.q[k].head, svc_read(P.q[k].tail));
-    for (int k = 0; k < 12; ++k) svc_write(P.error + k, 0u);
-    svc_write(S.live, 0u);
-    if (S.trace)
-    {
-      svc_write(S.trace, ~0ull);
-      for (int k = 1; k < 5; ++k) svc_write(S.trace + k, 0ull);
-    }
-    const unsigned long long *src = reinterpret_cast<const unsigned long long *>(&desc);
-    unsigned long long *dst = reinterpret_cast<unsigned long long *>(job);
-    for (uint32_t k = 0; k < sizeof(SvcJob) / 8; ++k)
-      if (k != 9) svc_write(dst + k, src[k]);
-    svc_write(&job->done, 0u);
-    svc_write(&job->remaining, SVC_BIAS);
-    asm volatile("s_waitcnt vmcnt(0)" ::: "memory");
-    svc_release();
+    sj_submit_begin(S, desc, defer);
   }
   __syncthreads();
   uint32_t mine = 0, tasks = 0;
@@ -1084,3 +1117,65 @@
     if (atomicAdd(&job->remaining, add) + add == 0u) svc_done(P, job, desc.epoch);
   }
 }
+
+__global__ __launch_bounds__(256) void k_defer_copy(const uint32_t *__restrict__ defer, uint32_t cap, const uint32_t *__restrict__ key, const uint32_t *__restrict__ idx,
+                                                    const uint32_t *__restrict__ src, uint32_t n, uint32_t *__restrict__ skey, uint32_t *__restrict__ sidx,
+                                                    uint32_t *__restrict__ soff, uint32_t *heavy, const uint32_t *__restrict__ gof, uint32_t heavy_min)
+{
+  const uint32_t cnt = min(defer[0], cap), k = blockIdx.x;
+  if (k >= cnt) return;
+  uint32_t off = 0;
+  for (uint32_t j = 0; j < k; ++j) off += defer[3 + 2 * j] - defer[2 + 2 * j];
+  const uint32_t first = defer[2 + 2 * k], last = defer[3 + 2 * k];
+  if (first >= last || last > n || off + (last - first) > n) return;
+  const uint32_t m = last - first;
+  if (threadIdx.x == 0)
+  {
+    soff[k] = off;
+    if (heavy && m > heavy_min) atomicMax(heavy + gof[first], m);
+  }
+  for (uint32_t i = threadIdx.x; i < m; i += blockDim.x)
+  {
+    skey[off + i] = key[first + i];
+    const uint32_t x = idx[first + i];
+    sidx[off + i] = src ? src[x] : x;
+  }
+}
+__global__ __launch_bounds__(256) void k_sort_job_submit_heaps(const SjParams S, const SvcJob desc, const uint32_t *__restrict__ defer, uint32_t cap, const uint32_t *__restrict__ soff)
+{
+  __shared__ uint32_t s_total;
+  const SvcParams &P = S.P;
+  SvcJob *job = P.jobs;
+  const uint32_t job_tag = desc.epoch << 8;
+  if (threadIdx.x == 0)
+  {
+    s_total = 0;
+    sj_submit_begin(S, desc, nullptr);
+  }
+  __syncthreads();
+  const uint32_t cnt = min(defer[0], cap);
+  uint32_t mine = 0;
+  for (uint32_t k = threadIdx.x; k < cnt; k += blockDim.x)
+  {
+    const uint32_t m = defer[3 + 2 * k] - defer[2 + 2 * k];
+    mine += m;
+    svc_push_heap(P, job, job_tag, soff[k], soff[k] + m);
+  }
+  atomicAdd(&s_total, mine);
+  __syncthreads();
+  if (threadIdx.x == 0)
+  {
+    const uint32_t add = s_total - SVC_BIAS;
+    if (atomicAdd(&job->remaining, add) + add == 0u) svc_done(P, job, desc.epoch);
+  }
+}
+__global__ void k_sort_job_stash(const uint32_t *error, const SvcJob *job, uint32_t *err)
+{
+  if (threadIdx.x < 12) err[threadIdx.x] = error[threadIdx.x];
+  if (threadIdx.x == 12) err[12] = job->remaining;
+}
+__global__ __launch_bounds__(256) void k_copy_u32(const uint32_t *__restrict__ src, uint32_t *__restrict__ dst, uint32_t m)
+{
+  const uint32_t i = blockIdx.x * blockDim.x + threadIdx.x;
+  if (i < m) dst[i] = src[i];
+}
diff --git a/include/breakid_hip.h b/include/breakid_hip.h
--- a/include/breakid_hip.h
+++ b/include/breakid_hip.h
@@ -380,6 +380,9 @@
 
 int bk_debug_std_sort(bk_ctx *ctx, const uint32_t *key, const uint64_t *group_off, uint32_t n_groups, uint32_t *perm_out);
 
+int bk_debug_defer_sort(bk_ctx *ctx, const uint32_t *key, const uint64_t *group_off, uint32_t n_groups, uint32_t defer_min, uint32_t defer_cap, uint32_t *perm_out,
+                        uint32_t *key_out, uint64_t out[6]);
+
 int bk_debug_scan(bk_ctx *ctx, int elem_bytes, const void *in, uint64_t n, int in_place, void *out);
 int bk_debug_radix_sort(bk_ctx *ctx, const uint64_t *keys, const uint32_t *vals, uint64_t n, int begin_bit, int end_bit, uint64_t *keys_out, uint32_t *vals_out);
 int bk_debug_prims_info(uint64_t out[4]);
```

Measured after the change: 11930 (median of 6 runs). 1.5% higher.
